# ZeldaM1/PnP-VCVE

Measured on NVIDIA B200. Metric: enhanced_frames_per_sec_720p, higher is better.
Workload: dtype bf16

## Files before the change

### pnpvcve_b200/csrc/pnp_api.cu

```cuda
#include <cmath>
#include <cstddef>
#include <cuda.h>
#include <cuda_runtime.h>
#include <mutex>
#include <stdio.h>
#include <stdlib.h>
#include <string.h>

#include "../../include/pnp_vcve.h"
#include "pnp_conv.cuh"
#include "pnp_ops.cuh"

namespace {

thread_local char g_err[512] = "";
int g_pair_override = -1;

static_assert(sizeof(pnp_dyn_entry) == sizeof(pnp::DynEntry), "launch-table entry layout");

int fail(int code, const char* fmt, const char* detail = "") {
  snprintf(g_err, sizeof(g_err), fmt, detail);
  return code;
}

int cuda_fail(cudaError_t e, const char* where) {
  snprintf(g_err, sizeof(g_err), "%s: %s", where, cudaGetErrorString(e));
  return PNP_ERR_CUDA;
}

struct DeviceInfo {
  bool ok = false;
  int sms = 0;
  int max_pairs = 0;
  cudaError_t err = cudaSuccess;
};

DeviceInfo g_dev[64];
std::once_flag g_dev_once[64];

int device_info(DeviceInfo** out) {
  int dev = 0;
  cudaError_t e = cudaGetDevice(&dev);
  if (e != cudaSuccess) return cuda_fail(e, "cudaGetDevice");
  if (dev < 0 || dev >= 64) return fail(PNP_ERR_ARG, "device ordinal out of range");
  std::call_once(g_dev_once[dev], [dev]() {
    cudaDeviceProp prop;
    cudaError_t e2 = cudaGetDeviceProperties(&prop, dev);
    if (e2 == cudaSuccess) {
      g_dev[dev].ok = (prop.major == 10);
      g_dev[dev].sms = prop.multiProcessorCount;
      if (g_dev[dev].ok) e2 = pnp::conv_rows_prepare(&g_dev[dev].max_pairs);
      if (g_dev[dev].ok && e2 == cudaSuccess) e2 = pnp::warp_prepare();
    }
    g_dev[dev].err = e2;
  });
  *out = &g_dev[dev];
  if (g_dev[dev].err != cudaSuccess) return cuda_fail(g_dev[dev].err, "device initialisation");
  if (!g_dev[dev].ok) return fail(PNP_ERR_ARCH, "libpnpvcve needs an sm_100 device (B200)");
  return PNP_OK;
}

struct Knobs {
  int l2_hints = 0;
  int par_split = 1;
  int warp_tma = 1;
  int pair = 0;
  int rings_nio = 0, rings_sa = 0;
  int debug_skip = 0;
  long long* trace = nullptr;
};

const Knobs& knobs() {
  static const Knobs k = []() {
    Knobs v;
    if (const char* e = getenv("PNP_L2_HINTS")) v.l2_hints = atoi(e);
    if (const char* e = getenv("PNP_PAR_SPLIT")) v.par_split = atoi(e) != 0;
    if (const char* e = getenv("PNP_PAIR")) v.pair = atoi(e);
    if (const char* e = getenv("PNP_WARP_TMA")) v.warp_tma = atoi(e) != 0;
    if (const char* e = getenv("PNP_RINGS")) {
      if (sscanf(e, "%d,%d", &v.rings_nio, &v.rings_sa) != 2) v.rings_nio = v.rings_sa = 0;
    }
#ifdef PNP_DIAG
    if (const char* e = getenv("PNP_DEBUG_SKIP")) v.debug_skip = atoi(e);
    if (const char* e = getenv("PNP_TRACE_PTR")) v.trace = reinterpret_cast<long long*>(strtoull(e, nullptr, 10));
#endif
    return v;
  }();
  return k;
}

pnp::DynRef dyn_ref(const pnp_dyn_ref* d) {
  pnp::DynRef r;
  r.table = d ? reinterpret_cast<const pnp::DynEntry*>(d->table) : nullptr;
  r.step = d ? d->step : nullptr;
  r.node = d ? d->node : 0;
  r.stride = d ? d->stride : 0;
  return r;
}

typedef CUresult (*MemsetD32AsyncFn)(CUdeviceptr, unsigned int, size_t, CUstream);

MemsetD32AsyncFn memset32_fn() {
  static MemsetD32AsyncFn fn = []() -> MemsetD32AsyncFn {
    void* p = nullptr;
    cudaDriverEntryPointQueryResult q;
    if (cudaGetDriverEntryPoint("cuMemsetD32Async", &p, cudaEnableDefault, &q) == cudaSuccess &&
        q == cudaDriverEntryPointSuccess)
      return reinterpret_cast<MemsetD32AsyncFn>(p);
    return nullptr;
  }();
  return fn;
}

int store_step(int32_t* word, int32_t value, cudaStream_t stream) {
  MemsetD32AsyncFn fn = memset32_fn();
  if (fn == nullptr) return fail(PNP_ERR_CUDA, "cuMemsetD32Async entry point not available");
  CUresult r = fn(reinterpret_cast<CUdeviceptr>(word), static_cast<unsigned int>(value), 1, stream);
  if (r != CUDA_SUCCESS) {
    snprintf(g_err, sizeof(g_err), "cuMemsetD32Async failed with CUresult %d", (int)r);
    return PNP_ERR_CUDA;
  }
  return PNP_OK;
}

typedef CUresult (*EncodeTiledFn)(CUtensorMap*, CUtensorMapDataType, cuuint32_t, void*, const cuuint64_t*,
                                  const cuuint64_t*, const cuuint32_t*, const cuuint32_t*,
                                  CUtensorMapInterleave, CUtensorMapSwizzle, CUtensorMapL2promotion,
                                  CUtensorMapFloatOOBfill);

EncodeTiledFn encode_fn() {
  static EncodeTiledFn fn = []() -> EncodeTiledFn {
    void* p = nullptr;
    cudaDriverEntryPointQueryResult q;
    if (cudaGetDriverEntryPoint("cuTensorMapEncodeTiled", &p, cudaEnableDefault, &q) == cudaSuccess &&
        q == cudaDriverEntryPointSuccess)
      return reinterpret_cast<EncodeTiledFn>(p);
    return nullptr;
  }();
  return fn;
}

int make_map(CUtensorMap* m, const void* base, int N, int H, int W, int box_w, long long spx = 0, long long sy = 0,
             long long sn = 0, int box_h = 1, int ch = 64) {
  EncodeTiledFn fn = encode_fn();
  if (fn == nullptr) return fail(PNP_ERR_CUDA, "cuTensorMapEncodeTiled entry point not available");
  const cuuint64_t px = (cuuint64_t)ch * 2;
  cuuint64_t dims[4] = {(cuuint64_t)ch, (cuuint64_t)W, (cuuint64_t)H, (cuuint64_t)N};
  cuuint64_t strides[3] = {px, (cuuint64_t)W * px, (cuuint64_t)H * W * px};
  if (spx != 0) {
    strides[0] = (cuuint64_t)spx * 2;
    strides[1] = (cuuint64_t)sy * 2;
    strides[2] = (cuuint64_t)sn * 2;
  }
  cuuint32_t box[4] = {(cuuint32_t)ch, (cuuint32_t)box_w, (cuuint32_t)box_h, 1};
  cuuint32_t estr[4] = {1, 1, 1, 1};
  CUresult r = fn(m, CU_TENSOR_MAP_DATA_TYPE_BFLOAT16, 4, const_cast<void*>(base), dims, strides, box, estr,
                  CU_TENSOR_MAP_INTERLEAVE_NONE, ch == 32 ? CU_TENSOR_MAP_SWIZZLE_64B : CU_TENSOR_MAP_SWIZZLE_128B,
                  CU_TENSOR_MAP_L2_PROMOTION_L2_256B,
                  CU_TENSOR_MAP_FLOAT_OOB_FILL_NONE);
  if (r != CUDA_SUCCESS) {
    snprintf(g_err, sizeof(g_err), "cuTensorMapEncodeTiled failed with CUresult %d", (int)r);
    return PNP_ERR_CUDA;
  }
  return PNP_OK;
}

bool aligned16(const void* p) { return (reinterpret_cast<uintptr_t>(p) & 15u) == 0; }

int frame_quality(const char* name, const void* a, bool a_u8, int64_t a_sf, int64_t a_sc, int64_t a_sy, const void* b,
                  bool b_u8, int64_t b_sf, int64_t b_sc, int64_t b_sy, int F, int H, int W, int crop_border,
                  unsigned long long* sse, double* ssim_sum, void* stream) {
  if (!a || !b || !sse || !ssim_sum) return fail(PNP_ERR_ARG, "%s: null pointer", name);
  if (F < 1 || crop_border < 0 || H - 2 * crop_border < 11 || W - 2 * crop_border < 11)
    return fail(PNP_ERR_ARG, "%s: the cropped frame must be at least 11 x 11", name);
  if ((long long)F * 3 > 65535) return fail(PNP_ERR_ARG, "%s: at most 21845 frames per call", name);
  DeviceInfo* d;
  int rc = device_info(&d);
  if (rc) return rc;
  double g[11], s = 0.0;
  for (int i = 0; i < 11; ++i) {
    g[i] = exp(-((double)(i - 5) * (i - 5)) / (2.0 * 1.5 * 1.5));
    s += g[i];
  }
  for (int i = 0; i < 11; ++i) g[i] /= s;
  const int ch_first = crop_border != 0 ? 2 : 0, n_ch = crop_border != 0 ? 1 : 3;
  cudaError_t e = pnp::launch_frame_quality(a, a_u8, a_sf, a_sc, a_sy, b, b_u8, b_sf, b_sc, b_sy, F, H, W, crop_border,
                                            ch_first, n_ch, g, sse, ssim_sum, d->sms, static_cast<cudaStream_t>(stream));
  return e == cudaSuccess ? PNP_OK : cuda_fail(e, name);
}

}

extern "C" {

static_assert(sizeof(pnp_conv_desc) == 280 && offsetof(pnp_conv_desc, out_spx) == 184 &&
                  offsetof(pnp_conv_desc, img_off) == 224 && offsetof(pnp_conv_desc, dyn) == 232 &&
                  offsetof(pnp_conv_desc, src_images) == 256 && offsetof(pnp_conv_desc, aux_channels) == 272 &&
                  offsetof(pnp_conv_desc, out_u8) == 276,
              "pnp_conv_desc layout is part of the ABI (mirrored by pnpvcve_b200/_lib.py: ConvDesc)");
int pnp_abi_version(void) { return 10; }

const char* pnp_last_error(void) { return g_err; }

int pnp_device_check(void) {
  DeviceInfo* d;
  return device_info(&d);
}

int pnp_device_pairs(void) {
  DeviceInfo* d;
  int rc = device_info(&d);
  return rc ? rc : d->max_pairs;
}

int pnp_set_pair_mode(int mode) {
  const int prev = g_pair_override;
  g_pair_override = mode < 0 ? -1 : (mode > 2 ? 2 : mode);
  return prev;
}

int pnp_graph_begin(void* stream) {
  DeviceInfo* d;
  int rc = device_info(&d);
  if (rc) return rc;
  cudaError_t e = cudaStreamBeginCapture(static_cast<cudaStream_t>(stream), cudaStreamCaptureModeRelaxed);
  return e == cudaSuccess ? PNP_OK : cuda_fail(e, "pnp_graph_begin");
}

int pnp_graph_end(void* stream, void** graph_exec) {
  if (!graph_exec) return fail(PNP_ERR_ARG, "pnp_graph_end: null output");
  *graph_exec = nullptr;
  cudaGraph_t g = nullptr;
  cudaError_t e = cudaStreamEndCapture(static_cast<cudaStream_t>(stream), &g);
  if (e != cudaSuccess || g == nullptr) {
    if (g) cudaGraphDestroy(g);
    return cuda_fail(e != cudaSuccess ? e : cudaErrorUnknown, "pnp_graph_end: capture");
  }
  cudaGraphExec_t x = nullptr;
  e = cudaGraphInstantiate(&x, g, 0);
  cudaGraphDestroy(g);
  if (e != cudaSuccess) return cuda_fail(e, "pnp_graph_end: instantiate");
  *graph_exec = x;
  return PNP_OK;
}

int pnp_graph_launch(void* graph_exec, int32_t* step_word, int32_t step_value, void* stream) {
  if (!graph_exec) return fail(PNP_ERR_ARG, "pnp_graph_launch: null graph");
  if (step_word) {
    int rc = store_step(step_word, step_value, static_cast<cudaStream_t>(stream));
    if (rc) return rc;
  }
  cudaError_t e = cudaGraphLaunch(static_cast<cudaGraphExec_t>(graph_exec), static_cast<cudaStream_t>(stream));
  return e == cudaSuccess ? PNP_OK : cuda_fail(e, "pnp_graph_launch");
}

int pnp_graph_destroy(void* graph_exec) {
  if (!graph_exec) return PNP_OK;
  cudaError_t e = cudaGraphExecDestroy(static_cast<cudaGraphExec_t>(graph_exec));
  return e == cudaSuccess ? PNP_OK : cuda_fail(e, "pnp_graph_destroy");
}

int pnp_set_step(int32_t* step_word, int32_t step_value, void* stream) {
  if (!step_word) return fail(PNP_ERR_ARG, "pnp_set_step: null step word");
  return store_step(step_word, step_value, static_cast<cudaStream_t>(stream));
}

int pnp_fetch_pinned(void* dst, const void* src_pinned, int64_t bytes, void* stream) {
  if (!dst || !src_pinned) return fail(PNP_ERR_ARG, "pnp_fetch_pinned: null pointer");
  if (bytes < 0 || (bytes & 15) || !aligned16(dst) || !aligned16(src_pinned))
    return fail(PNP_ERR_ARG, "pnp_fetch_pinned: size and pointers must be multiples of 16 bytes");
  DeviceInfo* d;
  int rc = device_info(&d);
  if (rc) return rc;
  cudaPointerAttributes at;
  cudaError_t e = cudaPointerGetAttributes(&at, src_pinned);
  if (e != cudaSuccess) return cuda_fail(e, "pnp_fetch_pinned");
  if (at.type != cudaMemoryTypeHost || at.devicePointer == nullptr)
    return fail(PNP_ERR_ARG, "pnp_fetch_pinned: src must be page-locked host memory the device can address");
  e = pnp::launch_fetch_pinned(at.devicePointer, dst, bytes, static_cast<cudaStream_t>(stream));
  return e == cudaSuccess ? PNP_OK : cuda_fail(e, "pnp_fetch_pinned");
}

int pnp_mv_warp(const void* src, const float* flow_x, const float* flow_y, int64_t flow_row_stride,
                int64_t flow_image_stride, void* dst, int N, int H, int W, int32_t* dbg_x0, int32_t* dbg_y0,
                void* stream) {
  if (!src || !flow_x || !flow_y || !dst) return fail(PNP_ERR_ARG, "pnp_mv_warp: null pointer");
  if (N <= 0 || H < 10 || W < 10) return fail(PNP_ERR_ARG, "pnp_mv_warp: bad shape (images of at least 10 x 10 pixels)");
  if (!aligned16(src) || !aligned16(dst) || src == dst)
    return fail(PNP_ERR_ARG, "pnp_mv_warp: src/dst must be distinct 16-byte aligned buffers");
  if ((dbg_x0 == nullptr) != (dbg_y0 == nullptr) || (dbg_x0 && N != 1))
    return fail(PNP_ERR_ARG, "pnp_mv_warp: dbg outputs come in pairs and need N == 1");
  DeviceInfo* d;
  int rc = device_info(&d);
  if (rc) return rc;
  CUtensorMap tm, tmd;
  if ((rc = make_map(&tm, src, N, H, W, 10, 0, 0, 0, 10))) return rc;
  if ((rc = make_map(&tmd, dst, N, H, W, 8, 0, 0, 0, 8))) return rc;
  cudaError_t e = pnp::launch_mv_warp(tm, tmd, src, flow_x, flow_y, flow_row_stride, flow_image_stride, dst, N, H, W, dbg_x0,
                                      dbg_y0, dyn_ref(nullptr), nullptr, knobs().warp_tma, static_cast<cudaStream_t>(stream));
  return e == cudaSuccess ? PNP_OK : cuda_fail(e, "pnp_mv_warp");
}

int pnp_mv_warp_dyn(const pnp_dyn_ref* dyn, const void* src_pool, int src_pool_images, int64_t flow_row_stride,
                    int64_t flow_image_stride, int N, int H, int W, void* stream) {
  if (!dyn || !dyn->table || !dyn->step) return fail(PNP_ERR_ARG, "pnp_mv_warp_dyn: null launch table");
  if (N <= 0 || H < 10 || W < 10) return fail(PNP_ERR_ARG, "pnp_mv_warp_dyn: bad shape (images of at least 10 x 10 pixels)");
  if (!src_pool || src_pool_images < N || !aligned16(src_pool))
    return fail(PNP_ERR_ARG, "pnp_mv_warp_dyn: src_pool must be the 16-byte aligned buffer every table entry's src lies in");
  DeviceInfo* d;
  int rc = device_info(&d);
  if (rc) return rc;
  CUtensorMap tm, tmd;
  if ((rc = make_map(&tm, src_pool, src_pool_images, H, W, 10, 0, 0, 0, 10))) return rc;
  if ((rc = make_map(&tmd, src_pool, src_pool_images, H, W, 8, 0, 0, 0, 8))) return rc;
  cudaError_t e = pnp::launch_mv_warp(tm, tmd, nullptr, nullptr, nullptr, flow_row_stride, flow_image_stride, nullptr, N, H, W,
                                      nullptr, nullptr, dyn_ref(dyn), src_pool, knobs().warp_tma,
                                      static_cast<cudaStream_t>(stream));
  return e == cudaSuccess ? PNP_OK : cuda_fail(e, "pnp_mv_warp_dyn");
}

int pnp_lr_im2col(const float* lr, int64_t sn, int64_t sc, int64_t sy, void* dst, int N, int H, int W,
                  int dst_channels, void* stream) {
  if (!lr || !dst) return fail(PNP_ERR_ARG, "pnp_lr_im2col: null pointer");
  if (N <= 0 || H <= 0 || W <= 0 || !aligned16(dst) || (dst_channels != 64 && dst_channels != 32))
    return fail(PNP_ERR_ARG, "pnp_lr_im2col: bad argument (dst_channels is 64 or 32)");
  DeviceInfo* d;
  int rc = device_info(&d);
  if (rc) return rc;
  cudaError_t e = pnp::launch_lr_im2col(lr, sn, sc, sy, dst, N, H, W, dst_channels, dyn_ref(nullptr),
                                        static_cast<cudaStream_t>(stream));
  return e == cudaSuccess ? PNP_OK : cuda_fail(e, "pnp_lr_im2col");
}

int pnp_lr_im2col_dyn(const pnp_dyn_ref* dyn, int64_t sn, int64_t sc, int64_t sy, int N, int H, int W, int dst_channels,
                      void* stream) {
  if (!dyn || !dyn->table || !dyn->step) return fail(PNP_ERR_ARG, "pnp_lr_im2col_dyn: null launch table");
  if (N <= 0 || H <= 0 || W <= 0 || (dst_channels != 64 && dst_channels != 32))
    return fail(PNP_ERR_ARG, "pnp_lr_im2col_dyn: bad shape (dst_channels is 64 or 32)");
  DeviceInfo* d;
  int rc = device_info(&d);
  if (rc) return rc;
  cudaError_t e = pnp::launch_lr_im2col(nullptr, sn, sc, sy, nullptr, N, H, W, dst_channels, dyn_ref(dyn),
                                        static_cast<cudaStream_t>(stream));
  return e == cudaSuccess ? PNP_OK : cuda_fail(e, "pnp_lr_im2col_dyn");
}

int pnp_pack_conv3x3_rowstack(const float* w, int n_experts, const float* coef, const float* row_scale,
                              int out_ch, int in_total, int in_begin, int in_begin2, int in_count, void* dst,
                              int tap_n, int flip_ky, void* stream) {
  if (!w || !dst) return fail(PNP_ERR_ARG, "pnp_pack_conv3x3_rowstack: null pointer");
  if (n_experts < 1 || (coef == nullptr && n_experts != 1) || out_ch < 1 || (tap_n != 64 && tap_n != 16) ||
      out_ch > tap_n || in_count < 1 || in_count > 64 || in_begin < 0 || in_begin + in_count > in_total ||
      (in_begin2 >= 0 && in_begin2 + in_count > in_total) || !aligned16(dst))
    return fail(PNP_ERR_ARG, "pnp_pack_conv3x3_rowstack: bad argument");
  DeviceInfo* d;
  int rc = device_info(&d);
  if (rc) return rc;
  cudaError_t e = pnp::launch_pack_conv3x3_rowstack(w, n_experts, coef, row_scale, out_ch, in_total, in_begin, in_begin2,
                                                    in_count, dst, tap_n, flip_ky != 0, static_cast<cudaStream_t>(stream));
  return e == cudaSuccess ? PNP_OK : cuda_fail(e, "pnp_pack_conv3x3_rowstack");
}

int pnp_pack_rows(const float* w, int rows, int cols, int64_t row_stride, int64_t col_stride, void* dst,
                  int row_offset, void* stream) {
  if (!w || !dst) return fail(PNP_ERR_ARG, "pnp_pack_rows: null pointer");
  if (rows < 1 || rows > 64 || cols < 1 || cols > 64 || row_offset < 0 || !aligned16(dst))
    return fail(PNP_ERR_ARG, "pnp_pack_rows: bad argument");
  DeviceInfo* d;
  int rc = device_info(&d);
  if (rc) return rc;
  cudaError_t e = pnp::launch_pack_rows(w, rows, cols, row_stride, col_stride, dst, row_offset,
                                        static_cast<cudaStream_t>(stream));
  return e == cudaSuccess ? PNP_OK : cuda_fail(e, "pnp_pack_rows");
}

int pnp_pack_aux(const float* w, int out_ch, int in_total, void* dst, void* stream) {
  if (!w || !dst) return fail(PNP_ERR_ARG, "pnp_pack_aux: null pointer");
  if (out_ch < 1 || out_ch > 64 || in_total < 3 || !aligned16(dst))
    return fail(PNP_ERR_ARG, "pnp_pack_aux: bad argument");
  DeviceInfo* d;
  int rc = device_info(&d);
  if (rc) return rc;
  cudaError_t e = pnp::launch_pack_aux(w, out_ch, in_total, dst, static_cast<cudaStream_t>(stream));
  return e == cudaSuccess ? PNP_OK : cuda_fail(e, "pnp_pack_aux");
}

int pnp_pack_mix_blocks(const float* w2, const float* w1x1, int n_blocks, int n_experts, const float* coef,
                        const float* row_scale, void* dst, int64_t dst_block_stride, void* stream) {
  if (!w2 || !w1x1 || !coef || !row_scale || !dst) return fail(PNP_ERR_ARG, "pnp_pack_mix_blocks: null pointer");
  if (n_blocks < 1 || n_blocks > 65535 || n_experts < 1 || dst_block_stride < 12 * 8192 || (dst_block_stride & 15) ||
      !aligned16(dst))
    return fail(PNP_ERR_ARG, "pnp_pack_mix_blocks: bad argument");
  DeviceInfo* d;
  int rc = device_info(&d);
  if (rc) return rc;
  cudaError_t e = pnp::launch_pack_mix_blocks(w2, w1x1, n_blocks, n_experts, coef, row_scale, dst, dst_block_stride,
                                              static_cast<cudaStream_t>(stream));
  return e == cudaSuccess ? PNP_OK : cuda_fail(e, "pnp_pack_mix_blocks");
}

int pnp_caa_heads(const float* base_qp, const float* qp, int frames, const float* base0_w,
                  const float* base0_b, const float* base2_w, const float* base2_b, const float* se0_w,
                  const float* se2_w, int n_experts, int se_hidden, float* experts, float* gamma,
                  void* stream) {
  if (!base_qp || !qp || !base0_w || !base0_b || !base2_w || !base2_b || !se0_w || !se2_w || !experts || !gamma)
    return fail(PNP_ERR_ARG, "pnp_caa_heads: null pointer");
  if (frames < 1 || n_experts < 1 || n_experts > 16 || se_hidden < 1 || se_hidden > 64)
    return fail(PNP_ERR_ARG, "pnp_caa_heads: bad argument");
  DeviceInfo* d;
  int rc = device_info(&d);
  if (rc) return rc;
  cudaError_t e = pnp::launch_caa_heads(base_qp, qp, frames, base0_w, base0_b, base2_w, base2_b, se0_w, se2_w,
                                        n_experts, se_hidden, experts, gamma, static_cast<cudaStream_t>(stream));
  return e == cudaSuccess ? PNP_OK : cuda_fail(e, "pnp_caa_heads");
}

int pnp_mix_bias(const float* conv2_bias, int n_blocks, int n_experts, const float* experts,
                 const float* gamma, int frames, float* out, void* stream) {
  if (!conv2_bias || !experts || !gamma || !out) return fail(PNP_ERR_ARG, "pnp_mix_bias: null pointer");
  if (n_blocks < 1 || n_blocks > 65535 || n_experts < 1 || frames < 1)
    return fail(PNP_ERR_ARG, "pnp_mix_bias: bad argument");
  DeviceInfo* d;
  int rc = device_info(&d);
  if (rc) return rc;
  cudaError_t e = pnp::launch_mix_bias(conv2_bias, (long long)n_experts * 64, n_blocks, n_experts, experts, gamma,
                                       frames, out, static_cast<cudaStream_t>(stream));
  return e == cudaSuccess ? PNP_OK : cuda_fail(e, "pnp_mix_bias");
}

int pnp_mv_rasterize(const float* records, const int32_t* frame_offsets, const int32_t* is_b,
                     const int32_t* p_target, int T, int R, int H, int W, uint32_t* owner_fwd,
                     uint32_t* owner_bwd, uint32_t* part_mask, float* mvs, float* partitions,
                     int32_t* status, void* stream) {
  if (!frame_offsets || !is_b || !p_target || !owner_fwd || !owner_bwd || !part_mask || !mvs || !partitions ||
      !status || (R > 0 && !records))
    return fail(PNP_ERR_ARG, "pnp_mv_rasterize: null pointer");
  if (T < 1 || T > 65535 || R < 0 || H < 1 || H > 65535 || W < 1 || (long long)T * H * W >= (1LL << 31))
    return fail(PNP_ERR_ARG, "pnp_mv_rasterize: bad shape");
  DeviceInfo* d;
  int rc = device_info(&d);
  if (rc) return rc;
  cudaError_t e = pnp::launch_mv_rasterize(records, frame_offsets, is_b, p_target, T, R, H, W, owner_fwd, owner_bwd,
                                           part_mask, mvs, partitions, status, static_cast<cudaStream_t>(stream));
  return e == cudaSuccess ? PNP_OK : cuda_fail(e, "pnp_mv_rasterize");
}

int pnp_frame_quality(const float* a, int64_t a_sf, int64_t a_sc, int64_t a_sy, const float* b, int64_t b_sf,
                      int64_t b_sc, int64_t b_sy, int F, int H, int W, int crop_border, unsigned long long* sse,
                      double* ssim_sum, void* stream) {
  return frame_quality("pnp_frame_quality", a, false, a_sf, a_sc, a_sy, b, false, b_sf, b_sc, b_sy, F, H, W, crop_border,
                       sse, ssim_sum, stream);
}

int pnp_frame_quality_u8(const void* a, int a_is_u8, int64_t a_sf, int64_t a_sc, int64_t a_sy, const void* b,
                         int b_is_u8, int64_t b_sf, int64_t b_sc, int64_t b_sy, int F, int H, int W, int crop_border,
                         unsigned long long* sse, double* ssim_sum, void* stream) {
  return frame_quality("pnp_frame_quality_u8", a, a_is_u8 != 0, a_sf, a_sc, a_sy, b, b_is_u8 != 0, b_sf, b_sc, b_sy, F,
                       H, W, crop_border, sse, ssim_sum, stream);
}

int pnp_unit_from_u8(const uint8_t* src, int64_t s_sf, int64_t s_sc, int64_t s_sy, float* dst, int64_t d_sf,
                     int64_t d_sc, int64_t d_sy, int F, int H, int W, void* stream) {
  if (!src || !dst) return fail(PNP_ERR_ARG, "pnp_unit_from_u8: null pointer");
  if (F < 1 || F > 65535 || H < 1 || H > 21845 || W < 1)
    return fail(PNP_ERR_ARG, "pnp_unit_from_u8: bad shape (1 <= F <= 65535, 1 <= H <= 21845)");
  DeviceInfo* d;
  int rc = device_info(&d);
  if (rc) return rc;
  cudaError_t e = pnp::launch_unit_from_u8(src, s_sf, s_sc, s_sy, dst, d_sf, d_sc, d_sy, F, H, W,
                                           static_cast<cudaStream_t>(stream));
  return e == cudaSuccess ? PNP_OK : cuda_fail(e, "pnp_unit_from_u8");
}

int pnp_conv3x3(const pnp_conv_desc* c, void* stream) {
  if (!c) return fail(PNP_ERR_ARG, "pnp_conv3x3: null descriptor");
  const bool table = c->dyn.table != nullptr;
  if (!c->src || (!table && !c->wpack)) return fail(PNP_ERR_ARG, "pnp_conv3x3: null src/wpack");
  if (table && (!c->dyn.step || c->dyn.node < 0 || c->dyn.stride <= c->dyn.node))
    return fail(PNP_ERR_ARG, "pnp_conv3x3: bad launch-table reference");
  if (c->N < 1 || c->H < 8 || c->W < 1) return fail(PNP_ERR_ARG, "pnp_conv3x3: bad shape (at least 8 rows)");
  const bool last = (c->mode == PNP_CONV_LAST);
  if (c->mode != PNP_CONV_BF16 && !last) return fail(PNP_ERR_ARG, "pnp_conv3x3: bad mode");
  const bool par = c->par != nullptr;
  if (last) {
    if (!c->lq || !c->outf || c->tap_n != 16 || c->aux || c->idt || par)
      return fail(PNP_ERR_ARG, "pnp_conv3x3: PNP_CONV_LAST needs lq/outf, tap_n=16, no aux/idt/par");
  } else {
    if (!c->out || c->tap_n != 64) return fail(PNP_ERR_ARG, "pnp_conv3x3: PNP_CONV_BF16 needs out and tap_n=64");
    if (c->out == c->src && !table) return fail(PNP_ERR_ARG, "pnp_conv3x3: out must not alias src (halo rows)");
  }
  if ((c->aux != nullptr) != (c->aux_k16 > 0) || c->aux_k16 < 0 || c->aux_k16 > 4)
    return fail(PNP_ERR_ARG, "pnp_conv3x3: aux / aux_k16 mismatch");
  const bool aux32 = c->aux && c->aux_channels == 32;
  if (c->aux && c->aux_channels != 0 && c->aux_channels != 64 && !aux32)
    return fail(PNP_ERR_ARG, "pnp_conv3x3: aux_channels is 64 (or 0) or 32");
  if (aux32 && c->aux_k16 > 2) return fail(PNP_ERR_ARG, "pnp_conv3x3: a 32-channel aux source carries K <= 32");
  if (par && (c->aux || c->idt)) return fail(PNP_ERR_ARG, "pnp_conv3x3: par takes no aux / idt");
  if (c->act < 0 || c->act > 2) return fail(PNP_ERR_ARG, "pnp_conv3x3: bad act");
  const bool strided_out = c->out_spx != 0 || c->out_sy != 0 || c->out_sn != 0;
  if (strided_out && (last || c->out_spx < 64 || c->out_sy < c->out_spx * c->W || (c->N > 1 && c->out_sn < c->out_sy * c->H) ||
                      ((c->out_spx | c->out_sy | c->out_sn) & 7)))
    return fail(PNP_ERR_ARG, "pnp_conv3x3: out strides must be non-overlapping multiples of 8 elements (PNP_CONV_BF16 only)");
  if (c->out_u8 && !last) return fail(PNP_ERR_ARG, "pnp_conv3x3: out_u8 needs PNP_CONV_LAST");
  if (c->lq_up4 && (!last || (c->H & 3) || (c->W & 3)))
    return fail(PNP_ERR_ARG, "pnp_conv3x3: lq_up4 needs PNP_CONV_LAST and H, W multiples of 4");
  if (!aligned16(c->src) || (c->wpack && !aligned16(c->wpack)) || (c->aux && !aligned16(c->aux)) ||
      (c->idt && !aligned16(c->idt)) || (c->out && !aligned16(c->out)))
    return fail(PNP_ERR_ARG, "pnp_conv3x3: pointers must be 16-byte aligned");
  if (c->src_images < 0 || c->aux_images < 0 || c->idt_images < 0 || c->out_images < 0)
    return fail(PNP_ERR_ARG, "pnp_conv3x3: negative image count");
  DeviceInfo* d;
  int rc = device_info(&d);
  if (rc) return rc;
  if (c->per_image && (c->N > d->sms || (!table && !c->img_off)))
    return fail(PNP_ERR_ARG, "pnp_conv3x3: per_image needs img_off and at most one image per SM");

  const Knobs& kn = knobs();
  pnp::ConvParams p;
  memset(&p, 0, sizeof(p));
  auto images = [&](int32_t n) { return n > 0 ? n : c->N; };
  if ((rc = make_map(&p.tm_src, c->src, images(c->src_images), c->H, c->W, pnp::kHaloPx))) return rc;
  if (c->aux && (rc = make_map(&p.tm_aux, c->aux, images(c->aux_images), c->H, c->W, pnp::kTilePx, 0, 0, 0, 1,
                               aux32 ? 32 : 64)))
    return rc;
  if (c->idt && (rc = make_map(&p.tm_id, c->idt, images(c->idt_images), c->H, c->W, pnp::kTilePx))) return rc;
  if (!last && (rc = make_map(&p.tm_out, c->out, images(c->out_images), c->H, c->W, pnp::kTilePx, c->out_spx, c->out_sy,
                              c->out_sn)))
    return rc;
  if (last) p.tm_out = p.tm_src;
  p.dyn = dyn_ref(&c->dyn);
  p.wpack = c->wpack;
  p.scale = c->scale;
  p.bias = c->bias;
  p.has_bias = c->bias != nullptr;
  p.img_off = c->per_image ? reinterpret_cast<const long long*>(c->img_off) : nullptr;
  p.par = c->par;
  p.has_par = par ? 1 : 0;
  p.par_sn = c->par_sn; p.par_sc = c->par_sc; p.par_sy = c->par_sy;
  p.lq = c->lq;
  p.lq_sn = c->lq_sn; p.lq_sc = c->lq_sc; p.lq_sy = c->lq_sy;
  p.outf = c->outf;
  p.of_sn = c->of_sn; p.of_sc = c->of_sc; p.of_sy = c->of_sy;
  p.out_u8 = c->out_u8 ? 1 : 0;
  p.H = c->H; p.W = c->W; p.N = c->N;
  p.strips = (c->W + pnp::kTilePx - 1) / pnp::kTilePx;
  const long long tiles = (long long)c->N * p.strips * c->H;
  if (tiles > 0x7fffffffLL) return fail(PNP_ERR_ARG, "pnp_conv3x3: too many tiles");
  p.tiles_total = (int)tiles;
  const long long cols = (long long)c->N * p.strips;
  const int pair_mode = g_pair_override >= 0 ? g_pair_override : kn.pair;
  const bool pair_ok = pair_mode != 0 && !last && !aux32 && c->tap_n == 64 && d->max_pairs >= 8 && (!par || kn.par_split) &&
                       (c->per_image ? (p.strips % 2 == 0 && c->N <= d->max_pairs)
                                     : (cols % 2 == 0 || cols >= 15 || pair_mode == 2));
  int grid;
  if (pair_ok) {
    p.pair = 1;
    const int max_pairs = d->max_pairs < d->sms / 2 ? d->max_pairs : d->sms / 2;
    if (c->per_image) {
      const int tiles_img = (p.strips / 2) * c->H;
      int cpi = max_pairs / c->N;
      if (cpi > tiles_img) cpi = tiles_img;
      p.tiles_per_cta = (tiles_img + cpi - 1) / cpi;
      cpi = (tiles_img + p.tiles_per_cta - 1) / p.tiles_per_cta;
      p.cpi = cpi;
      p.tiles_total = tiles_img * c->N;
      grid = 2 * cpi * c->N;
    } else {
      const long long pair_tiles = ((cols + 1) / 2) * c->H;
      p.tiles_total = (int)pair_tiles;
      int clusters = max_pairs < pair_tiles ? max_pairs : (int)pair_tiles;
      p.tiles_per_cta = (p.tiles_total + clusters - 1) / clusters;
      clusters = (p.tiles_total + p.tiles_per_cta - 1) / p.tiles_per_cta;
      grid = 2 * clusters;
    }
  } else if (c->per_image) {
    const int tiles_img = p.strips * c->H;
    int cpi = d->sms / c->N;
    if (cpi > tiles_img) cpi = tiles_img;
    p.tiles_per_cta = (tiles_img + cpi - 1) / cpi;
    cpi = (tiles_img + p.tiles_per_cta - 1) / p.tiles_per_cta;
    p.cpi = cpi;
    grid = cpi * c->N;
  } else {
    grid = d->sms < p.tiles_total ? d->sms : p.tiles_total;
    p.tiles_per_cta = (p.tiles_total + grid - 1) / grid;
    grid = (p.tiles_total + p.tiles_per_cta - 1) / p.tiles_per_cta;
  }
  p.tap_n = c->tap_n;
  p.aux_k16 = c->aux_k16;
  p.aux_pitch64 = aux32 ? 1 : 0;
  p.has_id = c->idt != nullptr;
  p.act = c->act;
  p.mode = last ? pnp::kModeLast : pnp::kModeBf16;
  p.flip_y = c->flip_y ? 1 : 0;
  p.w_stable = c->wpack_stable ? 1 : 0;
  p.lq_up4 = c->lq_up4 ? 1 : 0;
  p.par_sparse = (par && c->par_sparse) ? 1 : 0;
  if (kn.l2_hints && c->idt && c->flip_y) {
    p.l2_src = p.l2_idt = 1;
    if (kn.l2_hints >= 2) p.l2_out = 2;
  } else if (kn.l2_hints >= 2 && par) {
    p.l2_src = kn.l2_hints == 2 ? 2 : 1;
    p.l2_out = kn.l2_hints == 2 ? 1 : 2;
  }
  p.par_split = (par && kn.par_split) ? 1 : 0;
  p.debug_skip = kn.debug_skip;
  p.trace = kn.trace;
  const long long budget = 232448 - 2048;
  const long long w_bytes = ((long long)9 * c->tap_n * 128 + (c->aux ? pnp::kWChunkBytes : 0) / (p.pair ? 2 : 1) +
                             (par ? 3 * 64 * 128 : 0) / (p.pair ? 2 : 1) + 1023) & ~1023LL;
  auto fixed_bytes = [&](int n_io) {
    return w_bytes + (c->aux ? 2 * pnp::kTileBytes : 0) + (long long)n_io * pnp::kTileBytes;
  };
  p.n_io = 2;
  if (par) p.n_io = 3;
  if (c->idt) {
    p.n_io = 4;
    while (p.n_io > 2 && (budget - fixed_bytes(p.n_io)) / pnp::kASlotBytes < 5) --p.n_io;
  }
  long long slots = (budget - fixed_bytes(p.n_io)) / pnp::kASlotBytes;
  const long long max_slots = 6;
  if (slots > max_slots) slots = max_slots;
  if (slots < 4) return fail(PNP_ERR_RESOURCE, "pnp_conv3x3: shared-memory budget cannot hold 4 source rows");
  if (c->idt && p.n_io < 3)
    return fail(PNP_ERR_RESOURCE, "pnp_conv3x3: idt needs 3 staging slots (drop aux)");
  p.s_a = (int)slots;
  if (kn.rings_nio >= 2 && kn.rings_nio <= pnp::kMaxIoSlots && kn.rings_sa >= 3 && kn.rings_sa <= pnp::kMaxASlots &&
      fixed_bytes(kn.rings_nio) + (long long)kn.rings_sa * pnp::kASlotBytes <= budget && !(c->idt && kn.rings_nio < 3) &&
      !(par && kn.rings_nio < 3)) {
    p.n_io = kn.rings_nio;
    p.s_a = kn.rings_sa;
  }
  cudaError_t e = pnp::launch_conv_rows(p, grid, static_cast<cudaStream_t>(stream));
  return e == cudaSuccess ? PNP_OK : cuda_fail(e, "pnp_conv3x3");
}

}
```

### pnpvcve_b200/csrc/pnp_conv.cuh

```cuda
#pragma once
#include <cuda.h>
#include <stdint.h>

namespace pnp {

constexpr int kTilePx = 128;
constexpr int kHaloPx = kTilePx + 2;
constexpr int kRowBytes = kHaloPx * 128;
constexpr int kASlotBytes = 17 * 1024;
constexpr int kTileBytes = kTilePx * 128;
constexpr int kWChunkBytes = 8192;
constexpr int kRowsThreads = 352;
constexpr int kRowsThreadsPar = 480;
constexpr int kEpilogueWarps = 8;
constexpr int kMaxASlots = 8;
constexpr int kMaxIoSlots = 6;
constexpr int kTmemCols = 512;

enum ConvMode { kModeBf16 = 0, kModeLast = 1 };
enum ConvAct { kActNone = 0, kActLrelu = 1, kActRelu = 2 };

struct DynEntry {
  unsigned long long p[6];
  int i[4];
};
static_assert(sizeof(DynEntry) == 64, "launch-table entry is 64 bytes (ABI)");

struct DynRef {
  const DynEntry* table;
  const int* step;
  int node, stride;
  __device__ __forceinline__ const DynEntry* entry() const {
    return table ? table + ((long long)(*step) * stride + node) : nullptr;
  }
};

struct ConvParams {
  CUtensorMap tm_src;
  CUtensorMap tm_aux;
  CUtensorMap tm_id;
  CUtensorMap tm_out;
  DynRef dyn;
  const void* wpack;
  const float* scale;
  const float* bias;
  const long long* img_off;
  const float* par;
  long long par_sn, par_sc, par_sy;
  const float* lq;
  long long lq_sn, lq_sc, lq_sy;
  float* outf;
  long long of_sn, of_sc, of_sy;
  int H, W, N, strips;
  int tiles_total, tiles_per_cta;
  int cpi;
  int has_par;
  int has_bias;
  int tap_n;
  int aux_k16;
  int aux_pitch64;
  int has_id;
  int act;
  int mode;
  int flip_y;
  int l2_src, l2_idt, l2_out;
  int par_split;
  int par_sparse;
  int lq_up4;
  int w_stable;
  int pair;
  int s_a;
  int n_io;
  long long* trace;
  int debug_skip;
  int out_u8;
};

__device__ __forceinline__ void par_sparse_select(float& p0, float& p1, float& p2) {
  const bool n2 = p2 != 0.f, n1 = p1 != 0.f, n0 = p0 != 0.f;
  const float c = 1.0f / 255.0f;
  p2 = n2 ? c : 0.f;
  p1 = (!n2 && n1) ? c : 0.f;
  p0 = (!n2 && !n1 && n0) ? c : 0.f;
}

size_t conv_rows_smem_bytes(const ConvParams& p);
cudaError_t conv_rows_prepare(int* max_pairs);
cudaError_t launch_conv_rows(const ConvParams& p, int grid, cudaStream_t stream);

}
```

### pnpvcve_b200/csrc/pnp_conv_rows.cu

```cuda
#include <type_traits>

#include "pnp_conv.cuh"
#include "pnp_ops.cuh"
#include "pnp_ptx.cuh"

#ifdef PNP_DIAG
#define PNP_DBG(bit) ((p.debug_skip & (bit)) != 0)
#define PNP_TRACING (p.trace != nullptr)
#else
#define PNP_DBG(bit) false
#define PNP_TRACING false
#endif

namespace pnp {

namespace {

constexpr int kAccRingMax = 8;
#ifndef PNP_STEP_RING_LOG2
#define PNP_STEP_RING_LOG2 4
#endif
constexpr int kStepShift = PNP_STEP_RING_LOG2;
constexpr int kStepRing = 1 << kStepShift;
constexpr int kParCol = 320;

struct RowsLayout {
  uint32_t w, a, aux, io, misc, total;
};

__host__ __device__ inline RowsLayout rows_layout(int w_bytes, int s_a, int has_aux, int n_io) {
  RowsLayout l;
  l.w = 0;
  l.a = l.w + ((w_bytes + 1023) & ~1023);
  l.aux = l.a + s_a * kASlotBytes;
  l.io = l.aux + (has_aux ? 2 * kTileBytes : 0);
  l.misc = l.io + n_io * kTileBytes;
  l.total = l.misc + 1024;
  return l;
}

struct RowsMisc {
  float scale[64];
  float bias[64];
  uint64_t w_full;
  uint64_t a_full[kMaxASlots];
  uint64_t step_done[kStepRing];
  uint64_t acc_free[kAccRingMax];
  uint64_t par_done;
  uint64_t aux_full[2];
  uint64_t id_full[kMaxIoSlots];
  uint64_t io_empty[kMaxIoSlots];
  uint32_t tmem_base;
  uint32_t go_step;
  uint32_t go_par;
  uint32_t slot_free;
  uint64_t dy_full[kMaxIoSlots];
  uint64_t peer_w;
};
static_assert(sizeof(RowsMisc) <= 1024, "misc region overflow");

struct Segment {
  int n, strip, y_b, len, j_first, j_last;
};

struct SegIter {
  int t, t_end, H, strips, n, strip, y_b, dcol;
  __device__ SegIter(const ConvParams& p, int b, int e, int rank = 0) : t(b), t_end(e), H(p.H), strips(p.strips) {
    int col = b / p.H;
    y_b = b - col * p.H;
    dcol = p.pair ? 2 : 1;
    if (p.pair) col = 2 * col + rank;
    n = col / p.strips;
    strip = col - n * p.strips;
  }
  __device__ __forceinline__ bool valid() const { return t < t_end; }
  __device__ __forceinline__ Segment get() const {
    Segment s;
    s.n = n;
    s.strip = strip;
    s.y_b = y_b;
    s.len = min(H - y_b, t_end - t);
    s.j_first = (y_b > 0) ? -1 : 0;
    s.j_last = (y_b + s.len < H) ? s.len : s.len - 1;
    return s;
  }
  __device__ __forceinline__ void next(const Segment& s) {
    t += s.len;
    y_b = 0;
    strip += dcol;
    while (strip >= strips) {
      strip -= strips;
      ++n;
    }
  }
};

struct Ring {
  uint32_t slot, phase, size;
  __device__ explicit Ring(uint32_t n) : slot(0), phase(0), size(n) {}
  __device__ __forceinline__ void advance() {
    if (++slot == size) {
      slot = 0;
      phase ^= 1;
    }
  }
};

__device__ __forceinline__ float act_fn(float v, int act) {
  if (act == kActLrelu) return v > 0.f ? v : 0.1f * v;
  if (act == kActRelu) return fmaxf(v, 0.f);
  return v;
}

}

template <bool kPar, bool kScale, bool kPair>
__global__ void __launch_bounds__(kPar ? kRowsThreadsPar : kRowsThreads, 1)
conv3x3_rows_kernel(const __grid_constant__ ConvParams p) {
  constexpr int kAccRing = kPar ? 5 : 8;
  const int rank = kPair ? (int)cluster_ctarank() : 0;
  const int unit = kPair ? (int)(blockIdx.x >> 1) : (int)blockIdx.x;
  extern __shared__ uint8_t smem_raw[];
  const uint32_t raw = smem_u32(smem_raw);
  const uint32_t sbase = (raw + 1023u) & ~1023u;
  uint8_t* sgen = smem_raw + (sbase - raw);
  const int tap_n = p.tap_n;
  const int dx_block_bytes = 3 * tap_n * 128;
  const int w_bytes = kPair ? 3 * dx_block_bytes + (p.aux_k16 > 0 ? kWChunkBytes / 2 : 0) + (kPar ? 3 * 64 * 128 / 2 : 0)
                            : 3 * dx_block_bytes + (p.aux_k16 > 0 ? kWChunkBytes : 0) + (kPar ? 3 * 64 * 128 : 0);
  const RowsLayout L = rows_layout(w_bytes, p.s_a, p.aux_k16 > 0, p.n_io);
  RowsMisc* misc = reinterpret_cast<RowsMisc*>(sgen + L.misc);

  const int warp = threadIdx.x >> 5;
  const int lane = threadIdx.x & 31;
  int t_begin, t_end, img = 0;
  if (p.cpi > 0) {
    img = unit / p.cpi;
    const int tiles_img = (kPair ? p.strips >> 1 : p.strips) * p.H;
    t_begin = img * tiles_img + (unit - img * p.cpi) * p.tiles_per_cta;
    t_end = min((img + 1) * tiles_img, t_begin + p.tiles_per_cta);
  } else {
    t_begin = unit * p.tiles_per_cta;
    t_end = min(p.tiles_total, t_begin + p.tiles_per_cta);
  }
  const DynEntry* dyn = p.dyn.entry();
  const long long* img_off = dyn ? reinterpret_cast<const long long*>(dyn->p[5]) : p.img_off;
  const long long w_off = img_off ? img_off[2 * img] : 0, b_off = img_off ? img_off[2 * img + 1] : 0;
  const uint8_t* const wpack = (dyn ? reinterpret_cast<const uint8_t*>(dyn->p[0]) : static_cast<const uint8_t*>(p.wpack)) + w_off;
  const float* const bias_g = p.has_bias ? (dyn ? reinterpret_cast<const float*>(dyn->p[1]) : p.bias) + b_off : nullptr;
  const float* const par_g = dyn ? reinterpret_cast<const float*>(dyn->p[2]) : p.par;
  const float* const lq_g = dyn ? reinterpret_cast<const float*>(dyn->p[3]) : p.lq;
  float* const outf_g = dyn ? reinterpret_cast<float*>(dyn->p[4]) : p.outf;
  const int src_f = dyn ? dyn->i[0] : 0, aux_f = dyn ? dyn->i[1] : 0, idt_f = dyn ? dyn->i[2] : 0,
            out_f = dyn ? dyn->i[3] : 0;
  const int s_a = p.s_a;
  const int n_io = p.n_io;
  const bool last_mode = (p.mode == kModeLast);
  const int y_flip_base = p.flip_y ? p.H - 1 : 0;
  const int y_sign = p.flip_y ? -1 : 1;
#define PNP_Y(yy) (y_flip_base + y_sign * (yy))

  if (threadIdx.x < 64) {
    misc->scale[threadIdx.x] = p.scale ? p.scale[threadIdx.x] : 1.0f;
    const int nb = last_mode ? 3 : 64;
    misc->bias[threadIdx.x] = (bias_g && threadIdx.x < nb) ? bias_g[threadIdx.x] : 0.0f;
  }
  if (warp == 0) {
    if (lane == 0) {
      mbar_init(smem_u32(&misc->w_full), 1);
      for (int i = 0; i < kMaxASlots; ++i) mbar_init(smem_u32(&misc->a_full[i]), 1);
      for (int i = 0; i < kStepRing; ++i) mbar_init(smem_u32(&misc->step_done[i]), 1);
      const int acc_readers = kEpilogueWarps * (kPair ? 2 : 1);
      for (int i = 0; i < kAccRingMax; ++i) mbar_init(smem_u32(&misc->acc_free[i]), acc_readers);
      mbar_init(smem_u32(&misc->peer_w), 1);
      for (int i = 0; i < kMaxIoSlots; ++i) mbar_init(smem_u32(&misc->dy_full[i]), 4);
      misc->slot_free = 0;
      mbar_init(smem_u32(&misc->par_done), 1);
      for (int i = 0; i < 2; ++i) mbar_init(smem_u32(&misc->aux_full[i]), 1);
      for (int i = 0; i < kMaxIoSlots; ++i) {
        mbar_init(smem_u32(&misc->id_full[i]), 1);
        mbar_init(smem_u32(&misc->io_empty[i]), 1);
      }
      misc->go_step = 0;
      misc->go_par = 0;
      mbar_fence_init();
      tma_prefetch_desc(&p.tm_src);
      if (!last_mode) tma_prefetch_desc(&p.tm_out);
    }
    __syncwarp();
    if (kPair) tmem_alloc2(smem_u32(&misc->tmem_base), kTmemCols);
    else tmem_alloc(smem_u32(&misc->tmem_base), kTmemCols);
  }
  tc_fence_before();
  if (kPair) cluster_sync_all(); else __syncthreads();
  tc_fence_after();
  const uint32_t tmem_base = misc->tmem_base;
  griddep_launch_dependents();
  const uint32_t w_smem_early = sbase + L.w;
  auto load_weights = [&]() {
    const uint32_t wbar = smem_u32(&misc->w_full);
    mbar_arrive_expect_tx(wbar, w_bytes);
    if (kPair) {
      const int h192 = dx_block_bytes >> 1, h64 = (tap_n * 128) >> 1;
      for (int dx = 0; dx < 3; ++dx)
        bulk_load_1d(w_smem_early + dx * h192, wpack + dx * dx_block_bytes + rank * h192, h192, wbar);
      for (int b = 0; b < 9; ++b)
        bulk_load_1d(w_smem_early + 3 * h192 + b * h64, wpack + b * (tap_n * 128) + rank * h64, h64, wbar);
      const int extra = w_bytes - 3 * dx_block_bytes;
      if (extra > 0)
        bulk_load_1d(w_smem_early + 3 * dx_block_bytes, wpack + 3 * dx_block_bytes + rank * extra, extra, wbar);
    } else {
      for (int off = 0; off < w_bytes; off += kWChunkBytes) {
        const int n = min(kWChunkBytes, w_bytes - off);
        bulk_load_1d(w_smem_early + off, wpack + off, n, wbar);
      }
    }
  };
  if (p.w_stable && warp == 0) {
    if (elect_one()) load_weights();
    __syncwarp();
  }
  griddep_wait();
  if (PNP_TRACING && threadIdx.x == 0) {
    p.trace[2048 + blockIdx.x] = -clock64();
    p.trace[2208 + blockIdx.x] = (long long)globaltimer_ns();
  }
  const bool par_defer = kPar && p.par_split && PNP_DBG(1024);
  const bool hot_waits = !PNP_DBG(32);
  const uint32_t hint_ns = PNP_DBG(64) ? 40u : 200u;
  auto pwait = [&](uint32_t bar, uint32_t parity, int tag) {
    if (hot_waits) mbar_wait(bar, parity, tag); else mbar_wait_patient(bar, parity, tag, hint_ns);
  };
  auto ewait = [&](uint32_t bar, uint32_t parity, int tag) {
    if (hot_waits) mbar_wait(bar, parity, tag); else mbar_wait_warp(bar, parity, tag, hint_ns);
  };
  auto slow_epilogue = [&]() {
    if (PNP_DBG(2048)) __nanosleep(2000);
  };
  const uint32_t w_smem = sbase + L.w;
  const uint32_t a_smem = sbase + L.a;
  const uint32_t aux_smem = sbase + L.aux;
  const uint32_t io_smem = sbase + L.io;

  if (warp == 0) {
    if (elect_one()) {
      if (!p.w_stable) load_weights();
      const uint64_t pol_src = p.l2_src == 2 ? l2_policy_evict_last() : l2_policy_evict_first();
      Ring ar(s_a);
      uint32_t sc = 0, ord = 0;
      uint32_t aux_step[2] = {0, 0};
      for (SegIter it(p, t_begin, t_end, rank); it.valid();) {
        const Segment s = it.get();
        const int x0 = s.strip * kTilePx;
        for (int j = s.j_first; j <= s.j_last; ++j, ++sc, ar.advance()) {
          if (sc >= (uint32_t)s_a) {
            const uint32_t ps = sc - s_a + (par_defer ? 1u : 0u);
            pwait(smem_u32(&misc->step_done[ps & (kStepRing - 1)]), (ps >> kStepShift) & 1, 1);
          }
          const uint32_t fb = smem_u32(&misc->a_full[ar.slot]);
          if (kPair) {
            if (rank == 0) mbar_arrive_expect_tx(fb, 2 * kRowBytes);
            tma_load_4d_pair(a_smem + ar.slot * kASlotBytes, &p.tm_src, mapa_shared(fb, 0), 0, x0 - 1, PNP_Y(s.y_b + j),
                             s.n + src_f);
          } else if (PNP_DBG(1) && sc >= (uint32_t)s_a) {
            mbar_arrive(fb);
          } else {
            mbar_arrive_expect_tx(fb, kRowBytes);
            if (p.l2_src)
              tma_load_4d_hint(a_smem + ar.slot * kASlotBytes, &p.tm_src, fb, 0, x0 - 1, PNP_Y(s.y_b + j), s.n + src_f, pol_src);
            else
              tma_load_4d(a_smem + ar.slot * kASlotBytes, &p.tm_src, fb, 0, x0 - 1, PNP_Y(s.y_b + j), s.n + src_f);
          }
          if (j >= 0 && j < s.len) {
            if (p.aux_k16 > 0) {
              const uint32_t as = ord & 1;
              if (ord >= 2) {
                const uint32_t ps = aux_step[as];
                pwait(smem_u32(&misc->step_done[ps & (kStepRing - 1)]), (ps >> kStepShift) & 1, 2);
              }
              aux_step[as] = sc;
              const uint32_t ab = smem_u32(&misc->aux_full[as]);
              if (kPair) {
                if (rank == 0) mbar_arrive_expect_tx(ab, 2 * kTileBytes);
                tma_load_4d_pair(aux_smem + as * kTileBytes, &p.tm_aux, mapa_shared(ab, 0), 0, x0, PNP_Y(s.y_b + j),
                                 s.n + aux_f);
              } else {
                mbar_arrive_expect_tx(ab, p.aux_pitch64 ? kTileBytes / 2 : kTileBytes);
                tma_load_4d(aux_smem + as * kTileBytes, &p.tm_aux, ab, 0, x0, PNP_Y(s.y_b + j), s.n + aux_f);
              }
            }
            ++ord;
          }
        }
        it.next(s);
      }
    }
  } else if (warp == 1) {
    if (kPair && rank != 0) {
      if (elect_one()) {
        mbar_wait(smem_u32(&misc->w_full), 0, 4);
        mbar_arrive_cluster(mapa_shared(smem_u32(&misc->peer_w), 0));
      }
    } else if (elect_one()) {
      const uint32_t idesc0 = umma_idesc_bf16(kPair ? 256 : 128, 0);
      const uint32_t idesc_step = ((uint32_t)tap_n >> 3) << 17;
      const uint32_t w_lo = umma_desc_lo(w_smem);
      const uint32_t dxb = (uint32_t)dx_block_bytes >> 4;
      const uint32_t sbb = (uint32_t)(tap_n * 128) >> 4;
      const uint32_t aux_w_lo = w_lo + 3 * dxb;
      const uint32_t aux_a_hi = p.aux_pitch64 ? kDescHiSw64 : kDescHiSw128;
      const uint32_t par_w_lo = w_lo + 3 * dxb;
      const uint32_t u192 = dxb >> 1, u64 = sbb >> 1, w64_lo = w_lo + 3 * (dxb >> 1);
      mbar_wait(smem_u32(&misc->w_full), 0, 4);
      if (kPair) mbar_wait(smem_u32(&misc->peer_w), 0, 14);
      struct StepCtx {
        bool valid;
        int j, len, j_first;
        uint32_t ord0, sc, a_slot, a_phase;
      };
      SegIter seg_it(p, t_begin, t_end, rank);
      Segment seg = seg_it.valid() ? seg_it.get() : Segment{0, 0, 0, 0, 0, -1};
      Ring ar(s_a);
      StepCtx cur{seg_it.valid(), seg.j_first, seg.len, seg.j_first, 0u, 0u, ar.slot, ar.phase};
      auto advance = [&](StepCtx& c) {
        ar.advance();
        c.sc += 1;
        c.a_slot = ar.slot;
        c.a_phase = ar.phase;
        if (c.j < seg.j_last) {
          c.j += 1;
          return;
        }
        const uint32_t next_ord0 = c.ord0 + (uint32_t)seg.len;
        seg_it.next(seg);
        c.valid = seg_it.valid();
        if (c.valid) {
          seg = seg_it.get();
          c.j = seg.j_first;
          c.len = seg.len;
          c.j_first = seg.j_first;
          c.ord0 = next_ord0;
        }
      };
      auto ranges = [](const StepCtx& c, int& lo, int& cnt, int& old_cnt) {
        lo = max(c.j - 1, 0);
        const int hi = min(c.j + 1, c.len - 1);
        cnt = hi - lo + 1;
        const int new_from = (c.j == c.j_first) ? lo : c.j + 1;
        old_cnt = min(max(new_from - lo, 0), cnt);
      };
      const uint32_t go_step = smem_u32(&misc->go_step), go_par = smem_u32(&misc->go_par);
      bool pend = false;
      uint32_t pend_bar = 0;
      auto commit = [&](uint32_t bar) {
        if (kPair) umma2_commit(bar); else umma_commit(bar);
      };

      auto mma_range = [&](auto wrap_tag, uint32_t slot_lo, int cnt, uint32_t a_lo, uint32_t b_lo, uint32_t acc) {
        constexpr bool kWrap = decltype(wrap_tag)::value;
        if constexpr (!kWrap) {
          umma_bf16_lo(tmem_base + slot_lo * tap_n, a_lo, kDescHiSw128, b_lo, kDescHiSw128, idesc0 + cnt * idesc_step, acc);
        } else {
          const int n1 = min(cnt, kAccRing - (int)slot_lo);
          if (cnt > n1) {
            umma1_bf16_lo<1>(tmem_base + slot_lo * tap_n, a_lo, b_lo, idesc0 + n1 * idesc_step, acc);
            umma1_bf16_lo<3>(tmem_base, a_lo, b_lo + n1 * sbb, idesc0 + (cnt - n1) * idesc_step, acc);
          } else {
            umma_bf16_lo(tmem_base + slot_lo * tap_n, a_lo, kDescHiSw128, b_lo, kDescHiSw128, idesc0 + n1 * idesc_step, acc);
          }
        }
      };

      bool ppend = false;
      uint32_t pp_arow = 0, pp_od = 0;
      auto issue_par = [&](uint32_t a_row_, uint32_t od) {
        const uint32_t readers = (p.par_split ? 4u : (uint32_t)kEpilogueWarps) * (kPair ? 2u : 1u);
        if (kPair) {
          uint32_t spins = 0;
          while (ld_volatile_shared(go_par) < readers * od) {
            if (++spins > PNP_SPIN_LIMIT) {
              printf("pnp: flag wait timed out (tag 10, block %d, target %u)\n", (int)blockIdx.x, readers * od);
              __trap();
            }
          }
        } else {
          spin_until_ge(go_par, readers * od, 10);
        }
        tc_fence_after();
#pragma unroll
        for (int k = 0; k < 4; ++k) {
          if (kPair)
            umma2_bf16_lo<0>(tmem_base + kParCol, a_row_ + 8 + 2 * k, par_w_lo + 2 * k, idesc0 + 3 * idesc_step, k > 0);
          else
            umma_bf16_lo(tmem_base + kParCol, a_row_ + 8 + 2 * k, kDescHiSw128, par_w_lo + 2 * k, kDescHiSw128,
                         idesc0 + 3 * idesc_step, k > 0);
        }
        commit(smem_u32(&misc->par_done));
      };

      uint32_t go_seen = 0;
      const bool dbg_nopoll = PNP_DBG(8), dbg_nofence = PNP_DBG(16);
      if (cur.valid) go_seen = spin_until_ge_v(go_step, 1, 5);
      tc_fence_after();
      while (cur.valid) {
        const bool tr = PNP_TRACING && blockIdx.x == 0 && cur.sc < 64 && !PNP_DBG(128);
        if (tr) p.trace[cur.sc * 8 + 0] = clock64();
        int lo, cnt, old_cnt;
        ranges(cur, lo, cnt, old_cnt);
        const int new_cnt = cnt - old_cnt;
        const bool centre = (cur.j >= 0 && cur.j < cur.len);
        const uint32_t slot_lo = (cur.ord0 + lo) % kAccRing;
        const uint32_t a_row = umma_desc_lo(a_smem + cur.a_slot * kASlotBytes);
        const uint32_t sb_lo = (uint32_t)(lo - (cur.j - 1));
        const uint32_t b_row = w_lo + sb_lo * sbb;
        const uint32_t cur_sc = cur.sc;
        const uint32_t cur_od = cur.ord0 + (uint32_t)max(cur.j, 0);
        StepCtx nxt = cur;
        advance(nxt);
        auto step_body = [&](auto emit) {
#pragma unroll
          for (int dx = 0; dx < 3; ++dx) {
            if (kPar && dx == 1 && ppend) {
              issue_par(pp_arow, pp_od);
              ppend = false;
            }
            if (tr && dx == 1) p.trace[cur_sc * 8 + 6] = clock64();
            if (dx == 2) {
              if (tr) p.trace[cur_sc * 8 + 7] = clock64();
              if (nxt.valid && go_seen < nxt.sc + 1 && !dbg_nopoll) {
                go_seen = spin_until_ge_v(go_step, nxt.sc + 1, 5);
                if (!dbg_nofence) tc_fence_after();
              }
              if (tr) p.trace[cur_sc * 8 + 2] = clock64();
            }
#pragma unroll
            for (int k = 0; k < 4; ++k) {
              emit(dx, k);
              if (dx == 0 && k == 0 && pend) {
                commit(pend_bar);
                pend = false;
              }
              if (tr) p.trace[1024 + cur_sc * 16 + dx * 4 + k] = clock64();
            }
          }
        };
        if constexpr (kPair) {
          uint32_t dcol[3];
#pragma unroll
          for (int i = 0; i < 3; ++i) {
            uint32_t sl = slot_lo + (uint32_t)i;
            if (sl >= (uint32_t)kAccRing) sl -= (uint32_t)kAccRing;
            dcol[i] = tmem_base + sl * tap_n;
          }
          const uint32_t idesc_sb = idesc0 + idesc_step, idesc_win = idesc0 + 3 * idesc_step;
          auto rows = [&](auto cnt_tag, int dx, int k, uint32_t a_lo, bool first) {
            constexpr int kCnt = decltype(cnt_tag)::value;
            const uint32_t b0 = w64_lo + ((uint32_t)dx * 3 + sb_lo) * u64 + 2 * k;
            const uint32_t acc0 = first ? (old_cnt > 0) : 1u, acc1 = first ? (old_cnt > 1) : 1u,
                           acc2 = first ? (old_cnt > 2) : 1u;
            if constexpr (kCnt == 1) {
              umma2_bf16_lo<0>(dcol[0], a_lo, b0, idesc_sb, acc0);
            } else if constexpr (kCnt == 2) {
              umma2_bf16_lo<1>(dcol[0], a_lo, b0, idesc_sb, acc0);
              umma2_bf16_lo<3>(dcol[1], a_lo, b0 + u64, idesc_sb, acc1);
            } else {
              umma2_bf16_lo<1>(dcol[0], a_lo, b0, idesc_sb, acc0);
              umma2_bf16_lo<2>(dcol[1], a_lo, b0 + u64, idesc_sb, acc1);
              umma2_bf16_lo<3>(dcol[2], a_lo, b0 + 2 * u64, idesc_sb, acc2);
            }
          };
          if (cnt == 3 && slot_lo + 3u <= (uint32_t)kAccRing) {
            step_body([&](int dx, int k) {
              const uint32_t a_lo = a_row + dx * 8 + 2 * k;
              if (dx == 0 && k == 0) rows(std::integral_constant<int, 3>{}, dx, k, a_lo, true);
              else umma2_bf16_lo<0>(dcol[0], a_lo, w_lo + (uint32_t)dx * u192 + 2 * k, idesc_win, 1);
            });
          } else if (cnt == 3) {
            step_body([&](int dx, int k) {
              rows(std::integral_constant<int, 3>{}, dx, k, a_row + dx * 8 + 2 * k, dx == 0 && k == 0);
            });
          } else if (cnt == 2) {
            step_body([&](int dx, int k) {
              rows(std::integral_constant<int, 2>{}, dx, k, a_row + dx * 8 + 2 * k, dx == 0 && k == 0);
            });
          } else {
            step_body([&](int dx, int k) {
              rows(std::integral_constant<int, 1>{}, dx, k, a_row + dx * 8 + 2 * k, dx == 0 && k == 0);
            });
          }
        } else {
          auto emit1 = [&](auto wrap_tag, int dx, int k) {
            const uint32_t a_lo = a_row + dx * 8 + 2 * k;
            const uint32_t b_lo = b_row + dx * dxb + 2 * k;
            if (dx == 0 && k == 0) {
              if (old_cnt > 0) mma_range(wrap_tag, slot_lo, old_cnt, a_lo, b_lo, 1);
              if (new_cnt > 0)
                mma_range(wrap_tag, (slot_lo + old_cnt) % kAccRing, new_cnt, a_lo, b_lo + old_cnt * sbb, 0);
            } else {
              mma_range(wrap_tag, slot_lo, cnt, a_lo, b_lo, 1);
            }
          };
          if (slot_lo + (uint32_t)cnt > (uint32_t)kAccRing)
            step_body([&](int dx, int k) { emit1(std::true_type{}, dx, k); });
          else
            step_body([&](int dx, int k) { emit1(std::false_type{}, dx, k); });
        }
        if (p.aux_k16 > 0 && centre) {
          const uint32_t a_lo = umma_desc_lo(aux_smem + (cur_od & 1) * kTileBytes);
          for (int k = 0; k < p.aux_k16; ++k) {
            if (kPair)
              umma2_bf16_lo<0>(tmem_base + (cur_od % kAccRing) * tap_n, a_lo + 2 * k, aux_w_lo + 2 * k,
                               idesc0 + idesc_step, 1);
            else
              umma_bf16_lo(tmem_base + (cur_od % kAccRing) * tap_n, a_lo + 2 * k, aux_a_hi,
                           aux_w_lo + 2 * k, kDescHiSw128, idesc0 + idesc_step, 1);
          }
        }
        if (kPar && centre) {
          if (par_defer) {
            ppend = true;
            pp_arow = a_row;
            pp_od = cur_od;
          } else {
            issue_par(a_row, cur_od);
          }
        }
        pend = true;
        pend_bar = smem_u32(&misc->step_done[cur_sc & (kStepRing - 1)]);
        if (tr) p.trace[cur_sc * 8 + 1] = clock64();
        cur = nxt;
      }
      if (kPar && ppend) issue_par(pp_arow, pp_od);
      if (pend) commit(pend_bar);
    }
  } else if (warp == 10) {
    if ((!kPair || rank == 0) && elect_one()) {
      const uint32_t go_step = smem_u32(&misc->go_step);
      Ring ar(s_a);
      uint32_t sc = 0, ord0 = 0;
      for (SegIter it(p, t_begin, t_end, rank); it.valid();) {
        const Segment s = it.get();
        for (int j = s.j_first; j <= s.j_last; ++j, ++sc, ar.advance()) {
          const bool trs = PNP_TRACING && blockIdx.x == 0 && sc < 64;
          if (trs) p.trace[2560 + sc * 4 + 0] = clock64();
          mbar_wait(smem_u32(&misc->a_full[ar.slot]), ar.phase, 5);
          if (trs) p.trace[2560 + sc * 4 + 1] = clock64();
          const int lo = max(j - 1, 0), hi = min(j + 1, s.len - 1);
          const int new_from = (j == s.j_first) ? lo : j + 1;
          for (int o = max(new_from, lo); o <= hi; ++o) {
            const uint32_t od = ord0 + o;
            mbar_wait(smem_u32(&misc->acc_free[od % kAccRing]), ((od / kAccRing) & 1) ^ 1, 6);
          }
          const bool centre = (j >= 0 && j < s.len);
          if (p.aux_k16 > 0 && centre) {
            const uint32_t od = ord0 + j;
            mbar_wait(smem_u32(&misc->aux_full[od & 1]), (od >> 1) & 1, 7);
          }
          st_release_shared(go_step, sc + 1);
          if (trs) p.trace[2560 + sc * 4 + 2] = clock64();
        }
        ord0 += s.len;
        it.next(s);
      }
    }
  } else if (warp >= 11 && !(kPar && p.par_split)) {
  } else {
    const int q = warp & 3;
    const int half = (warp - 2) >> 2;
    const int row = q * 32 + lane;
    const bool store_warp = (warp == 2);
    const uint32_t sw = (uint32_t)(row & 7);
    const uint32_t lane_base = tmem_base + ((uint32_t)(q * 32) << 16);
    float bias_r[kPar ? 1 : 32], scale_r[(kScale && !kPar) ? 32 : 1];
    if (!kPar) {
#pragma unroll
      for (int j = 0; j < 32; ++j) {
        bias_r[j] = misc->bias[half * 32 + j];
        if (kScale) scale_r[j] = misc->scale[half * 32 + j];
      }
    }

    struct TileCur {
      SegIter it;
      Segment s;
      int o;
      uint32_t ord, sc0;
      bool valid;
    };
    TileCur cur{SegIter(p, t_begin, t_end, rank), Segment{0, 0, 0, 0, 0, -1}, 0, 0u, 0u, false};
    cur.valid = cur.it.valid();
    if (cur.valid) cur.s = cur.it.get();
    const uint32_t acc_free0 = kPair ? mapa_shared(smem_u32(&misc->acc_free[0]), 0) : smem_u32(&misc->acc_free[0]);
    const uint32_t go_par_a = kPair ? mapa_shared(smem_u32(&misc->go_par), 0) : smem_u32(&misc->go_par);
    auto acc_release = [&](uint32_t slot) {
      __syncwarp();
      if (lane == 0) {
        if (kPair) mbar_arrive_cluster(acc_free0 + slot * 8);
        else mbar_arrive(acc_free0 + slot * 8);
      }
    };
    auto par_release = [&]() {
      __syncwarp();
      if (lane == 0) {
        if (kPair) red_add_cluster(go_par_a);
        else asm volatile("red.relaxed.cta.shared::cta.add.u32 [%0], 1;" ::"r"(go_par_a) : "memory");
      }
    };
    auto phantom = [&](const Segment& sg) { return kPair && sg.n >= p.N; };
    auto tile_next = [](TileCur& c) {
      ++c.ord;
      if (++c.o < c.s.len) return;
      c.sc0 += (uint32_t)(c.s.j_last - c.s.j_first + 1);
      c.it.next(c.s);
      c.valid = c.it.valid();
      c.o = 0;
      if (c.valid) c.s = c.it.get();
    };

    auto blend_store = [&](uint8_t* slot_row, float q0, float q1, float q2) {
      if (p.par_sparse) par_sparse_select(q0, q1, q2);
#pragma unroll
      for (int gg = 0; gg < 2; ++gg) {
        float a1[16], a2[16], a3[16];
        const uint32_t col = kParCol + half * 32 + gg * 16;
        tmem_ld16(lane_base + col, a1);
        tmem_ld16(lane_base + col + 64, a2);
        tmem_ld16(lane_base + col + 128, a3);
        tmem_ld_wait();
        uint32_t w[8];
#pragma unroll
        for (int j = 0; j < 8; ++j)
          w[j] = pack_bf16x2(fmaf(q2, a3[2 * j], fmaf(q1, a2[2 * j], q0 * a1[2 * j])),
                             fmaf(q2, a3[2 * j + 1], fmaf(q1, a2[2 * j + 1], q0 * a1[2 * j + 1])));
        const int g = half * 2 + gg;
        *reinterpret_cast<uint4*>(slot_row + (((2 * g) ^ sw) << 4)) = make_uint4(w[0], w[1], w[2], w[3]);
        *reinterpret_cast<uint4*>(slot_row + (((2 * g + 1) ^ sw) << 4)) = make_uint4(w[4], w[5], w[6], w[7]);
      }
    };
    auto par_load = [&](const TileCur& c, float& q0, float& q1, float& q2) {
      const int x = c.s.strip * kTilePx + row;
      q0 = q1 = q2 = 0.f;
      if (x < p.W && !phantom(c.s)) {
        const float* pp = par_g + (long long)c.s.n * p.par_sn + (long long)PNP_Y(c.s.y_b + c.o) * p.par_sy + x;
        q0 = __ldg(pp);
        q1 = __ldg(pp + p.par_sc);
        q2 = __ldg(pp + 2 * p.par_sc);
      }
    };
    if (kPar && p.par_split) {
      const uint32_t slot_free = smem_u32(&misc->slot_free);
      if (warp >= 11) {
        float pn0 = 0.f, pn1 = 0.f, pn2 = 0.f;
        if (cur.valid) par_load(cur, pn0, pn1, pn2);
        Ring sl(n_io);
        while (cur.valid) {
          TileCur nxt = cur;
          tile_next(nxt);
          float pf0 = 0.f, pf1 = 0.f, pf2 = 0.f;
          if (nxt.valid) par_load(nxt, pf0, pf1, pf2);
          const bool trr = PNP_TRACING && blockIdx.x == 0 && cur.ord < 64 && warp == 11 && lane == 0;
          if (trr) p.trace[3072 + cur.ord * 4 + 0] = clock64();
          mbar_wait(smem_u32(&misc->par_done), cur.ord & 1, 11);
          if (trr) p.trace[3072 + cur.ord * 4 + 1] = clock64();
          tc_fence_after();
          if (p.par_sparse) par_sparse_select(pn0, pn1, pn2);
          uint32_t wv[32];
#pragma unroll
          for (int b4 = 0; b4 < 4; ++b4) {
            float a1[16], a2[16], a3[16];
            const uint32_t col = kParCol + b4 * 16;
            tmem_ld16(lane_base + col, a1);
            tmem_ld16(lane_base + col + 64, a2);
            tmem_ld16(lane_base + col + 128, a3);
            tmem_ld_wait();
            if (b4 == 3) {
              tc_fence_before();
              par_release();
              if (trr) p.trace[3072 + cur.ord * 4 + 2] = clock64();
            }
#pragma unroll
            for (int j = 0; j < 8; ++j)
              wv[b4 * 8 + j] = pack_bf16x2(fmaf(pn2, a3[2 * j], fmaf(pn1, a2[2 * j], pn0 * a1[2 * j])),
                                           fmaf(pn2, a3[2 * j + 1], fmaf(pn1, a2[2 * j + 1], pn0 * a1[2 * j + 1])));
          }
          if (cur.ord >= (uint32_t)n_io) spin_until_ge(slot_free, cur.ord - (uint32_t)n_io + 1, 12);
          uint8_t* rowp = sgen + L.io + sl.slot * kTileBytes + row * 128;
#pragma unroll
          for (int c8 = 0; c8 < 8; ++c8)
            *reinterpret_cast<uint4*>(rowp + ((c8 ^ sw) << 4)) =
                make_uint4(wv[4 * c8], wv[4 * c8 + 1], wv[4 * c8 + 2], wv[4 * c8 + 3]);
          warp_arrive(smem_u32(&misc->dy_full[sl.slot]));
          if (trr) p.trace[3072 + cur.ord * 4 + 3] = clock64();
          sl.advance();
          pn0 = pf0;
          pn1 = pf1;
          pn2 = pf2;
          cur = nxt;
        }
      } else {
        Ring ior(n_io);
        while (cur.valid) {
          const Segment& s = cur.s;
          const uint32_t ord = cur.ord;
          const int y = PNP_Y(s.y_b + cur.o);
          const uint32_t sc_last = cur.sc0 + (uint32_t)(min(cur.o + 1, s.j_last) - s.j_first);
          const uint32_t slot = ord % kAccRing;
          const uint32_t taddr = lane_base + slot * tap_n;
          if (store_warp) {
            if (elect_one()) {
              tma_store_wait_read<1>();
              if (ord >= 1) st_release_shared(slot_free, ord - 1);
            }
            __syncwarp();
          }
          const bool trm = PNP_TRACING && blockIdx.x == 0 && ord < 64 && warp == 2 && lane == 0;
          if (trm) p.trace[2816 + ord * 4 + 0] = clock64();
          slow_epilogue();
          mbar_wait(smem_u32(&misc->step_done[sc_last & (kStepRing - 1)]), (sc_last >> kStepShift) & 1, 9);
          if (trm) p.trace[2816 + ord * 4 + 1] = clock64();
          tc_fence_after();
          float v[32];
          tmem_ld16(taddr + half * 32, v);
          tmem_ld16(taddr + half * 32 + 16, v + 16);
          tmem_ld_wait();
          tc_fence_before();
          acc_release(slot);
          if (trm) p.trace[2816 + ord * 4 + 2] = clock64();
          mbar_wait(smem_u32(&misc->dy_full[ior.slot]), ior.phase, 13);
          if (trm) p.trace[2816 + ord * 4 + 3] = clock64();
          uint8_t* rowp = sgen + L.io + ior.slot * kTileBytes + row * 128;
#pragma unroll
          for (int gg = 0; gg < 2; ++gg) {
            const int g = half * 2 + gg;
            float* vv = v + gg * 16;
            const float4* sc4 = reinterpret_cast<const float4*>(&misc->scale[g * 16]);
            const float4* bi4 = reinterpret_cast<const float4*>(&misc->bias[g * 16]);
#pragma unroll
            for (int j4 = 0; j4 < 4; ++j4) {
              const float4 sc = kScale ? sc4[j4] : make_float4(1.f, 1.f, 1.f, 1.f);
              const float4 bi = bi4[j4];
              vv[4 * j4 + 0] = fmaf(vv[4 * j4 + 0], sc.x, bi.x);
              vv[4 * j4 + 1] = fmaf(vv[4 * j4 + 1], sc.y, bi.y);
              vv[4 * j4 + 2] = fmaf(vv[4 * j4 + 2], sc.z, bi.z);
              vv[4 * j4 + 3] = fmaf(vv[4 * j4 + 3], sc.w, bi.w);
            }
            uint4* c0 = reinterpret_cast<uint4*>(rowp + (((2 * g) ^ sw) << 4));
            uint4* c1 = reinterpret_cast<uint4*>(rowp + (((2 * g + 1) ^ sw) << 4));
            const uint4 i0 = *c0, i1 = *c1;
            const uint32_t iw[8] = {i0.x, i0.y, i0.z, i0.w, i1.x, i1.y, i1.z, i1.w};
#pragma unroll
            for (int j = 0; j < 8; ++j) {
              vv[2 * j] += bf16_lo(iw[j]);
              vv[2 * j + 1] += bf16_hi(iw[j]);
            }
#pragma unroll
            for (int j = 0; j < 16; ++j) vv[j] = act_fn(vv[j], p.act);
            *c0 = make_uint4(pack_bf16x2(vv[0], vv[1]), pack_bf16x2(vv[2], vv[3]), pack_bf16x2(vv[4], vv[5]),
                             pack_bf16x2(vv[6], vv[7]));
            *c1 = make_uint4(pack_bf16x2(vv[8], vv[9]), pack_bf16x2(vv[10], vv[11]), pack_bf16x2(vv[12], vv[13]),
                             pack_bf16x2(vv[14], vv[15]));
          }
          fence_proxy_async_smem();
          named_bar_sync(2, 256);
          if (store_warp) {
            if (elect_one()) {
              if (!phantom(s)) {
                if (p.l2_out)
                  tma_store_4d_hint(&p.tm_out, io_smem + ior.slot * kTileBytes, 0, s.strip * kTilePx, y, s.n + out_f,
                                    p.l2_out == 2 ? l2_policy_evict_last() : l2_policy_evict_first());
                else
                  tma_store_4d(&p.tm_out, io_smem + ior.slot * kTileBytes, 0, s.strip * kTilePx, y, s.n + out_f);
              }
              tma_store_commit();
            }
            __syncwarp();
          }
          ior.advance();
          tile_next(cur);
        }
        if (store_warp) {
          if (elect_one()) tma_store_wait_all<0>();
          __syncwarp();
        }
      }
    } else {
    float pn0 = 0.f, pn1 = 0.f, pn2 = 0.f;
    if (kPar && cur.valid) {
      float q0, q1, q2;
      par_load(cur, q0, q1, q2);
      {
        TileCur n1 = cur;
        tile_next(n1);
        if (n1.valid) par_load(n1, pn0, pn1, pn2);
      }
      ewait(smem_u32(&misc->par_done), cur.ord & 1, 11);
      tc_fence_after();
      blend_store(sgen + L.io + row * 128, q0, q1, q2);
      tc_fence_before();
      par_release();
    }

    TileCur idc = cur;
    Ring idr(n_io);
    auto load_id = [&](const TileCur& c, uint32_t slot) {
      const uint32_t ib = smem_u32(&misc->id_full[slot]);
      mbar_arrive_expect_tx(ib, kTileBytes);
      if (p.l2_idt)
        tma_load_4d_hint(io_smem + slot * kTileBytes, &p.tm_id, ib, 0, c.s.strip * kTilePx, PNP_Y(c.s.y_b + c.o), c.s.n + idt_f,
                         p.l2_idt == 2 ? l2_policy_evict_last() : l2_policy_evict_first());
      else
        tma_load_4d(io_smem + slot * kTileBytes, &p.tm_id, ib, 0, c.s.strip * kTilePx, PNP_Y(c.s.y_b + c.o), c.s.n + idt_f);
    };
    if (p.has_id && store_warp) {
      if (elect_one()) {
        for (int i = 0; i < n_io && idc.valid; ++i) {
          load_id(idc, idr.slot);
          idr.advance();
          tile_next(idc);
        }
      }
      __syncwarp();
    }

    auto lq_fetch = [&](const TileCur& c, float* r) {
      r[0] = r[1] = r[2] = 0.f;
      if (!c.valid || half != 0) return;
      const int x = c.s.strip * kTilePx + row;
      const int y = PNP_Y(c.s.y_b + c.o);
      if (x >= p.W) return;
      if (p.lq_up4) {
        const int hl = p.H >> 2, wl = p.W >> 2;
        const float sy = fmaxf(0.25f * ((float)y + 0.5f) - 0.5f, 0.f), sx = fmaxf(0.25f * ((float)x + 0.5f) - 0.5f, 0.f);
        const int y0 = (int)sy, x0 = (int)sx;
        const int y1 = y0 + (y0 < hl - 1 ? 1 : 0), x1 = x0 + (x0 < wl - 1 ? 1 : 0);
        const float ly1 = sy - (float)y0, lx1 = sx - (float)x0;
        const float ly0 = 1.f - ly1, lx0 = 1.f - lx1;
        const float* b0 = lq_g + (long long)c.s.n * p.lq_sn + (long long)y0 * p.lq_sy;
        const float* b1 = lq_g + (long long)c.s.n * p.lq_sn + (long long)y1 * p.lq_sy;
#pragma unroll
        for (int ch = 0; ch < 3; ++ch) {
          const float* c0 = b0 + ch * p.lq_sc;
          const float* c1 = b1 + ch * p.lq_sc;
          r[ch] = ly0 * (lx0 * __ldg(c0 + x0) + lx1 * __ldg(c0 + x1)) + ly1 * (lx0 * __ldg(c1 + x0) + lx1 * __ldg(c1 + x1));
        }
      } else {
        const float* lp = lq_g + (long long)c.s.n * p.lq_sn + (long long)y * p.lq_sy + x;
        r[0] = __ldg(lp);
        r[1] = __ldg(lp + p.lq_sc);
        r[2] = __ldg(lp + 2 * p.lq_sc);
      }
    };
    float lq_a[3] = {0.f, 0.f, 0.f}, lq_b[3] = {0.f, 0.f, 0.f};
    if (last_mode) {
      lq_fetch(cur, lq_a);
      TileCur n1 = cur;
      if (n1.valid) tile_next(n1);
      lq_fetch(n1, lq_b);
    }

    Ring ior(n_io);
    while (cur.valid) {
      slow_epilogue();
      const Segment& s = cur.s;
      const int o = cur.o;
      const uint32_t ord = cur.ord;
      const int x = s.strip * kTilePx + row;
      const bool valid = x < p.W;
      const int y = PNP_Y(s.y_b + o);
      const uint32_t sc_last = cur.sc0 + (uint32_t)(min(o + 1, s.j_last) - s.j_first);
      const uint32_t slot = ord % kAccRing;
      const uint32_t taddr = lane_base + slot * tap_n;
      TileCur nxt = cur;
      tile_next(nxt);
      if (last_mode) {
        const float r0 = lq_a[0], r1 = lq_a[1], r2 = lq_a[2];
        {
          TileCur n2 = nxt;
          if (n2.valid) tile_next(n2);
          lq_a[0] = lq_b[0];
          lq_a[1] = lq_b[1];
          lq_a[2] = lq_b[2];
          lq_fetch(n2, lq_b);
        }
        ewait(smem_u32(&misc->step_done[sc_last & (kStepRing - 1)]), (sc_last >> kStepShift) & 1, 9);
        tc_fence_after();
        float v[16];
        if (half == 0) {
          tmem_ld16(taddr, v);
          tmem_ld_wait();
        }
        tc_fence_before();
        acc_release(slot);
        if (valid && half == 0) {
          const long long o_off = (long long)s.n * p.of_sn + (long long)y * p.of_sy + x;
          const float o0 = v[0] + misc->bias[0] + r0, o1 = v[1] + misc->bias[1] + r1, o2 = v[2] + misc->bias[2] + r2;
          if (!kPar && p.out_u8) {
            uint8_t* op = reinterpret_cast<uint8_t*>(outf_g) + o_off;
            op[0] = (uint8_t)quant_u8(o0);
            op[p.of_sc] = (uint8_t)quant_u8(o1);
            op[2 * p.of_sc] = (uint8_t)quant_u8(o2);
          } else {
            float* op = outf_g + o_off;
            op[0] = o0;
            op[p.of_sc] = o1;
            op[2 * p.of_sc] = o2;
          }
        }
        cur = nxt;
        continue;
      }
      const bool tr = PNP_TRACING && blockIdx.x == 0 && ord < 64 && threadIdx.x == 64 && !PNP_DBG(128);
      float pf0 = 0.f, pf1 = 0.f, pf2 = 0.f;
      if (kPar && nxt.valid) {
        TileCur n2 = nxt;
        tile_next(n2);
        if (n2.valid) par_load(n2, pf0, pf1, pf2);
      }
      const uint32_t s_io = ior.slot;
      if (store_warp) {
        if (elect_one()) {
          tma_store_wait_read<1>();
          if (p.has_id && ord >= 2 && idc.valid) {
            load_id(idc, idr.slot);
            idr.advance();
            tile_next(idc);
          }
        }
        __syncwarp();
      }
      if (p.has_id) {
        ewait(smem_u32(&misc->id_full[s_io]), ior.phase, 8);
      } else {
        named_bar_sync(1, 256);
      }
      if (kPar && nxt.valid) {
        ewait(smem_u32(&misc->par_done), (ord + 1) & 1, 11);
      } else {
        ewait(smem_u32(&misc->step_done[sc_last & (kStepRing - 1)]), (sc_last >> kStepShift) & 1, 9);
      }
      tc_fence_after();
      if (tr) p.trace[ord * 8 + 3] = clock64();
      uint8_t* rowp = sgen + L.io + s_io * kTileBytes + row * 128;
      float v[32];
      if (PNP_DBG(4)) {
#pragma unroll
        for (int j = 0; j < 32; ++j) v[j] = 0.f;
      } else {
        tmem_ld16(taddr + half * 32, v);
        tmem_ld16(taddr + half * 32 + 16, v + 16);
        if (kPar && nxt.valid) {
          const uint32_t s_nx = (s_io + 1 == (uint32_t)n_io) ? 0u : s_io + 1;
          blend_store(sgen + L.io + s_nx * kTileBytes + row * 128, pn0, pn1, pn2);
        } else {
          tmem_ld_wait();
        }
      }
      tc_fence_before();
      acc_release(slot);
      if (kPar && nxt.valid) par_release();
#pragma unroll
      for (int gg = 0; gg < 2; ++gg) {
        const int g = half * 2 + gg;
        float* vv = v + gg * 16;
        if (kPar) {
          const float4* sc4 = reinterpret_cast<const float4*>(&misc->scale[g * 16]);
          const float4* bi4 = reinterpret_cast<const float4*>(&misc->bias[g * 16]);
#pragma unroll
          for (int j4 = 0; j4 < 4; ++j4) {
            const float4 sc = kScale ? sc4[j4] : make_float4(1.f, 1.f, 1.f, 1.f);
            const float4 bi = bi4[j4];
            vv[4 * j4 + 0] = fmaf(vv[4 * j4 + 0], sc.x, bi.x);
            vv[4 * j4 + 1] = fmaf(vv[4 * j4 + 1], sc.y, bi.y);
            vv[4 * j4 + 2] = fmaf(vv[4 * j4 + 2], sc.z, bi.z);
            vv[4 * j4 + 3] = fmaf(vv[4 * j4 + 3], sc.w, bi.w);
          }
        } else {
#pragma unroll
          for (int j = 0; j < 16; ++j)
            vv[j] = kScale ? fmaf(vv[j], scale_r[gg * 16 + j], bias_r[gg * 16 + j]) : vv[j] + bias_r[gg * 16 + j];
        }
        uint4* c0 = reinterpret_cast<uint4*>(rowp + (((2 * g) ^ sw) << 4));
        uint4* c1 = reinterpret_cast<uint4*>(rowp + (((2 * g + 1) ^ sw) << 4));
        if (p.has_id || kPar) {
          const uint4 i0 = *c0, i1 = *c1;
          const uint32_t iw[8] = {i0.x, i0.y, i0.z, i0.w, i1.x, i1.y, i1.z, i1.w};
#pragma unroll
          for (int j = 0; j < 8; ++j) {
            vv[2 * j] += bf16_lo(iw[j]);
            vv[2 * j + 1] += bf16_hi(iw[j]);
          }
        }
#pragma unroll
        for (int j = 0; j < 16; ++j) vv[j] = act_fn(vv[j], p.act);
        uint4 o0, o1;
        o0.x = pack_bf16x2(vv[0], vv[1]);
        o0.y = pack_bf16x2(vv[2], vv[3]);
        o0.z = pack_bf16x2(vv[4], vv[5]);
        o0.w = pack_bf16x2(vv[6], vv[7]);
        o1.x = pack_bf16x2(vv[8], vv[9]);
        o1.y = pack_bf16x2(vv[10], vv[11]);
        o1.z = pack_bf16x2(vv[12], vv[13]);
        o1.w = pack_bf16x2(vv[14], vv[15]);
        if (!PNP_DBG(2)) {
          *c0 = o0;
          *c1 = o1;
        }
      }
      if (tr) p.trace[ord * 8 + 4] = clock64();
      fence_proxy_async_smem();
      named_bar_sync(2, 256);
      if (tr) p.trace[ord * 8 + 5] = clock64();
      if (store_warp) {
        if (elect_one()) {
          if (!PNP_DBG(2)) {
            if (!phantom(s)) {
              if (p.l2_out)
                tma_store_4d_hint(&p.tm_out, io_smem + s_io * kTileBytes, 0, s.strip * kTilePx, y, s.n + out_f,
                                  p.l2_out == 2 ? l2_policy_evict_last() : l2_policy_evict_first());
              else
                tma_store_4d(&p.tm_out, io_smem + s_io * kTileBytes, 0, s.strip * kTilePx, y, s.n + out_f);
            }
            tma_store_commit();
          }
        }
        __syncwarp();
      }
      ior.advance();
      if (kPar) {
        pn0 = pf0;
        pn1 = pf1;
        pn2 = pf2;
      }
      cur = nxt;
    }
    if (store_warp) {
      if (elect_one()) tma_store_wait_all<0>();
      __syncwarp();
    }
    }
  }

  tc_fence_before();
  if (kPair) cluster_sync_all(); else __syncthreads();
  if (PNP_TRACING && threadIdx.x == 0) {
    p.trace[2048 + blockIdx.x] += clock64();
    p.trace[2368 + blockIdx.x] = (long long)globaltimer_ns();
  }
  if (warp == 0) {
    tc_fence_after();
    if (kPair) tmem_dealloc2(tmem_base, kTmemCols);
    else tmem_dealloc(tmem_base, kTmemCols);
  }
}

#undef PNP_Y

size_t conv_rows_smem_bytes(const ConvParams& p) {
  const int full = 3 * 3 * p.tap_n * 128;
  const int w_bytes = p.pair ? full + (p.aux_k16 > 0 ? kWChunkBytes / 2 : 0) + (p.has_par ? 3 * 64 * 128 / 2 : 0)
                             : full + (p.aux_k16 > 0 ? kWChunkBytes : 0) + (p.has_par ? 3 * 64 * 128 : 0);
  return rows_layout(w_bytes, p.s_a, p.aux_k16 > 0, p.n_io).total + 1024;
}

namespace {
constexpr int kMaxSmem = 232448;

template <bool kPar, bool kScale, bool kPair>
cudaError_t launch_rows_variant(const ConvParams& p, int grid, size_t smem, cudaStream_t stream) {
  cudaLaunchConfig_t cfg = {};
  cfg.gridDim = dim3(grid);
  cfg.blockDim = dim3(kPar ? kRowsThreadsPar : kRowsThreads);
  cfg.dynamicSmemBytes = smem;
  cfg.stream = stream;
  cudaLaunchAttribute attr[2];
  attr[0].id = cudaLaunchAttributeProgrammaticStreamSerialization;
  attr[0].val.programmaticStreamSerializationAllowed = 1;
  cfg.attrs = attr;
  cfg.numAttrs = 1;
  if (kPair) {
    attr[1].id = cudaLaunchAttributeClusterDimension;
    attr[1].val.clusterDim.x = 2;
    attr[1].val.clusterDim.y = 1;
    attr[1].val.clusterDim.z = 1;
    cfg.numAttrs = 2;
  }
  return cudaLaunchKernelEx(&cfg, conv3x3_rows_kernel<kPar, kScale, kPair>, p);
}
template <bool kPar, bool kScale, bool kPair>
cudaError_t prepare_variant(int* max_pairs) {
  cudaError_t e = cudaFuncSetAttribute(conv3x3_rows_kernel<kPar, kScale, kPair>, cudaFuncAttributeMaxDynamicSharedMemorySize,
                                       kMaxSmem);
  if (e != cudaSuccess || !kPair) return e;
  cudaLaunchConfig_t cfg = {};
  cfg.gridDim = dim3(2 * 148);
  cfg.blockDim = dim3(kPar ? kRowsThreadsPar : kRowsThreads);
  cfg.dynamicSmemBytes = kMaxSmem;
  cudaLaunchAttribute attr[1];
  attr[0].id = cudaLaunchAttributeClusterDimension;
  attr[0].val.clusterDim.x = 2;
  attr[0].val.clusterDim.y = 1;
  attr[0].val.clusterDim.z = 1;
  cfg.attrs = attr;
  cfg.numAttrs = 1;
  int n = 0;
  e = cudaOccupancyMaxActiveClusters(&n, conv3x3_rows_kernel<kPar, kScale, kPair>, &cfg);
  if (e == cudaSuccess && n < *max_pairs) *max_pairs = n;
  return e;
}
}

cudaError_t conv_rows_prepare(int* max_pairs) {
  cudaError_t e;
  int pairs = 1 << 30;
  if ((e = prepare_variant<true, true, false>(&pairs)) != cudaSuccess) return e;
  if ((e = prepare_variant<true, false, false>(&pairs)) != cudaSuccess) return e;
  if ((e = prepare_variant<false, true, false>(&pairs)) != cudaSuccess) return e;
  if ((e = prepare_variant<false, false, false>(&pairs)) != cudaSuccess) return e;
  if ((e = prepare_variant<true, true, true>(&pairs)) != cudaSuccess) return e;
  if ((e = prepare_variant<true, false, true>(&pairs)) != cudaSuccess) return e;
  if ((e = prepare_variant<false, true, true>(&pairs)) != cudaSuccess) return e;
  if ((e = prepare_variant<false, false, true>(&pairs)) != cudaSuccess) return e;
  if (max_pairs) *max_pairs = pairs == (1 << 30) ? 0 : pairs;
  return cudaSuccess;
}

cudaError_t launch_conv_rows(const ConvParams& p, int grid, cudaStream_t stream) {
  const size_t smem = conv_rows_smem_bytes(p);
  const bool par = p.has_par != 0, scale = (p.scale != nullptr);
  if (p.pair) {
    if (par) return scale ? launch_rows_variant<true, true, true>(p, grid, smem, stream)
                          : launch_rows_variant<true, false, true>(p, grid, smem, stream);
    return scale ? launch_rows_variant<false, true, true>(p, grid, smem, stream)
                 : launch_rows_variant<false, false, true>(p, grid, smem, stream);
  }
  if (par) return scale ? launch_rows_variant<true, true, false>(p, grid, smem, stream)
                        : launch_rows_variant<true, false, false>(p, grid, smem, stream);
  return scale ? launch_rows_variant<false, true, false>(p, grid, smem, stream)
               : launch_rows_variant<false, false, false>(p, grid, smem, stream);
}

}
```

### pnpvcve_b200/engine.py

```python
import ctypes
import os

import numpy as np
import torch
import torch.nn.functional as F

from . import _lib, ops
from .ops import PNP_ACT_LRELU, PNP_ACT_NONE, PNP_ACT_RELU

SLICE_I, SLICE_P = 73, 80
ROW_BYTES = 9 * 64 * 128
WORK = ("kw", "pa", "pb", "xa", "xb", "t", "hr", "zero")


def key_schedule(key_row):
    t = len(key_row)
    bwd, fwd = [-1] * t, [-1] * t
    nxt = -1
    for i in range(t - 1, -1, -1):
        bwd[i] = nxt
        if key_row[i]:
            nxt = i
    prv = -1
    for i in range(t):
        fwd[i] = prv
        if key_row[i]:
            prv = i
    return bwd, fwd


def keyframe_rows(slices_host):
    key = (slices_host == SLICE_I) | (slices_host == SLICE_P)
    key[:, 0] = True
    key[:, -1] = True
    return key.tolist()


def group_clips(key_rows, max_batch, batch=True):
    groups = []
    for b, row in enumerate(key_rows):
        if batch and groups and row == key_rows[groups[-1][0]] and groups[-1][1] - groups[-1][0] < max_batch:
            groups[-1][1] = b + 1
        else:
            groups.append([b, b + 1])
    return [tuple(g) for g in groups]


def step_variants(bwd_key, fwd_key):
    t = len(bwd_key)
    names = []
    for s in range(t):
        i = t - 1 - s
        names.append("b_last" if i == t - 1 else ("b_merged" if bwd_key[i] == i + 1 else "b_sep"))
    for i in range(t):
        names.append("f_first" if i == 0 else ("f_merged" if fwd_key[i] == i - 1 else "f_sep"))
    return names


class _Program:

    def __init__(self, n, t, h, w, dev, maxn, nb, vsr, table_steps, lr_once=False):
        self.key = (n, t, h, w, dev, maxn, nb, vsr, lr_once)
        self.n, self.t, self.h, self.w, self.dev, self.maxn, self.nb, self.vsr = n, t, h, w, dev, maxn, nb, vsr
        self.img_bytes = h * w * 128
        self.lr_once = lr_once
        self.lr = torch.zeros((t * n if lr_once else maxn, h, w, 32), dtype=torch.bfloat16, device=dev)
        self.lr_img_bytes = h * w * 64
        first_work = t * n
        self.pool_images = first_work + len(WORK) * maxn
        self.pool = torch.empty((self.pool_images, h, w, 64), dtype=torch.bfloat16, device=dev)
        self.feats = self.pool[: t * n].view(t, n, h, w, 64)
        self.work = {}
        for k, name in enumerate(WORK):
            f0 = first_work + k * maxn
            self.work[name] = (f0, self.pool[f0:f0 + maxn])
        self.work["zero"][1].zero_()
        if vsr:
            self.u1 = ops.new_feature(maxn, 2 * h, 2 * w, dev)
            self.u2 = ops.new_feature(maxn, 4 * h, 4 * w, dev)
            self.hr4 = ops.new_feature(maxn, 4 * h, 4 * w, dev)
        self.stride = 8 + 2 * nb + (8 if vsr else 0)
        self.table_steps = 0
        self.table = self.img_off = self.host_table = self.host_off = None
        self.nodes = {}
        self.graphs = {}
        self.ensure_table(table_steps)
        self.step_word = torch.zeros(1, dtype=torch.int32, device=dev)
        self.cap_stream = torch.cuda.Stream(device=dev)
        self.uploaded = None

    def ensure_table(self, steps):
        if steps <= self.table_steps:
            return
        steps = max(steps, 2 * self.t)
        self.release_graphs()
        self.nodes = {}
        self.table_steps = steps
        self.table = torch.zeros((steps, self.stride, _lib.DYN_ENTRY_WORDS), dtype=torch.int64, device=self.dev)
        self.img_off = torch.zeros((steps, self.maxn, 2), dtype=torch.int64, device=self.dev)
        self.host_table = torch.zeros((steps, self.stride, _lib.DYN_ENTRY_WORDS), dtype=torch.int64).pin_memory()
        self.host_off = torch.zeros((steps, self.maxn, 2), dtype=torch.int64).pin_memory()

    def release_graphs(self):
        graphs, self.graphs = getattr(self, "graphs", {}), {}
        if graphs:
            lib = _lib.load()
            for g in graphs.values():
                lib.pnp_graph_destroy(g)

    def __del__(self):
        try:
            self.release_graphs()
        except Exception:
            pass


class BaeEngine:

    def __init__(self, module):
        self.m = module
        self.static_key = None
        self.static = None
        self.mix_slots = {}
        self.mix_pool = None
        self.prog = None
        self.launch_count = 0
        self.last_mode = "graph"
        self._done = None
        self.prof = None
        self.prof_every = 1
        self.use_graphs = os.environ.get("PNP_GRAPHS", "1") != "0"
        self.batch_clips = os.environ.get("PNP_BATCH_CLIPS", "1") != "0"
        self.lr_once = {"0": False, "1": True}.get(os.environ.get("PNP_LR_ONCE", ""), None)
        self.max_batch = 16

    def _param_key(self):
        return tuple((id(p), p._version, p.device, p.data_ptr()) for p in self.m.parameters())

    def invalidate(self):
        self.static = self.static_key = None
        self.mix_slots = {}

    def __getstate__(self):
        return {"m": self.m}

    def __setstate__(self, state):
        self.__init__(state["m"])

    def _pack_static(self, dev):
        key = self._param_key()
        if self.static is not None and self.static_key == key:
            return self.static
        m = self.m
        nb = m.num_blocks
        st = {}

        def f32(p):
            return p.detach().to(dev, torch.float32).contiguous()

        conv1_w = torch.zeros((2 * nb, ROW_BYTES), dtype=torch.uint8, device=dev)
        conv1_b, c2w, c2b, w1x1 = [], [], [], []
        for br, (name, branch) in enumerate((("bwd", m.backward_resblocks), ("fwd", m.forward_resblocks))):
            w_in = f32(branch.input_conv[0].weight)
            st[name + "_in_bias"] = f32(branch.input_conv[0].bias)
            def pack(in_begin, in_begin2=-1, with_aux=False, w_in=w_in):
                buf = ops.new_wpack_rowstack(dev, with_aux=with_aux)
                ops.pack_conv3x3_rowstack(w_in, buf, in_begin=in_begin, in_begin2=in_begin2, in_count=64)
                if with_aux:
                    ops.pack_aux(w_in, buf[ROW_BYTES:])
                return buf
            if name == "bwd":
                st["bwd_key_aux"] = pack(3, with_aux=True)
                st["bwd_merged_aux"] = pack(3, 67, with_aux=True)
                st["bwd_nb"] = pack(67)
            else:
                st["fwd_bf_aux"] = pack(131, with_aux=True)
                st["fwd_key"] = pack(3)
                st["fwd_merged"] = pack(3, 67)
                st["fwd_nb"] = pack(67)
            for k, blk in enumerate(branch.main):
                ops.pack_conv3x3_rowstack(f32(blk.conv1.weight), conv1_w[br * nb + k], flip_ky=True)
                conv1_b.append(f32(blk.conv1.bias))
                c2w.append(f32(blk.conv2.weight))
                c2b.append(f32(blk.conv2.bias))
                w1x1.append(torch.stack([f32(c.weight).view(64, 64) for c in
                                         (blk.conv16x16, blk.conv16x8, blk.conv8x8)], 0))
        st["conv1_w"] = conv1_w
        st["conv1_b"] = torch.stack(conv1_b, 0).contiguous()
        st["conv2_w_all"] = torch.stack(c2w, 0).contiguous()
        st["w1x1_all"] = torch.stack(w1x1, 0).contiguous()
        st["conv2_bias_all"] = torch.stack(c2b, 0).contiguous()
        hr = ops.new_wpack_rowstack(dev)
        ops.pack_conv3x3_rowstack(f32(m.conv_hr.weight), hr)
        st["hr_w"], st["hr_b"] = hr, f32(m.conv_hr.bias)
        last = ops.new_wpack_rowstack(dev, tap_n=16)
        ops.pack_conv3x3_rowstack(f32(m.conv_last.weight), last, tap_n=16)
        st["last_w"], st["last_b"] = last, f32(m.conv_last.bias)
        if m.vsr:
            for name, mod in (("up1", m.upsample1), ("up2", m.upsample2)):
                w_up, b_up = f32(mod.upsample_conv.weight), f32(mod.upsample_conv.bias)
                packs, biases = [], []
                for g in range(4):
                    buf = ops.new_wpack_rowstack(dev)
                    ops.pack_conv3x3_rowstack(w_up[g::4].contiguous(), buf)
                    packs.append(buf)
                    biases.append(b_up[g::4].contiguous())
                st[name + "_w"], st[name + "_b"] = packs, biases
        st["caa"] = dict(b0w=f32(m.BasePredictor.BaseNet[0].weight), b0b=f32(m.BasePredictor.BaseNet[0].bias),
                         b2w=f32(m.BasePredictor.BaseNet[2].weight), b2b=f32(m.BasePredictor.BaseNet[2].bias),
                         s0w=f32(m.BiasePredictor.fc[0].weight), s2w=f32(m.BiasePredictor.fc[2].weight))
        st["nb"] = nb
        self.static, self.static_key = st, key
        self.mix_slots = {}
        return st

    def _mix_slots_for(self, st, conds, experts, gamma, dev):
        nb2 = 2 * st["nb"]
        pool = self.mix_pool
        if pool is not None and (pool.device != dev or pool.shape[1] != nb2):
            pool = self.mix_pool = None
            self.mix_slots = {}
        need = [c for c in conds if c not in self.mix_slots]
        cap = 0 if pool is None else pool.shape[0]
        if len(self.mix_slots) + len(need) > cap:
            if len(conds) > cap:
                self.mix_pool = None
                self.mix_pool = torch.empty((max(48, 2 * len(conds)), nb2, ops.PACK_A_BYTES), dtype=torch.uint8, device=dev)
            self.mix_slots = {}
            need = list(conds)
        for c in need:
            slot = len(self.mix_slots)
            f = conds[c]
            ops.pack_mix_blocks(st["conv2_w_all"], st["w1x1_all"], experts[f], gamma[f], self.mix_pool[slot])
            self.mix_slots[c] = slot
        return self.mix_slots

    def _program(self, n, t, h, w, dev, maxn, steps):
        extra = t * n * h * w * 64
        lr_once = self.lr_once if self.lr_once is not None else \
            extra <= torch.cuda.get_device_properties(dev).total_memory // 8
        key = (n, t, h, w, dev, maxn, self.m.num_blocks, bool(self.m.vsr), lr_once)
        if self.prog is None or self.prog.key != key:
            self.prog = None
            self.prog = _Program(n, t, h, w, dev, maxn, self.m.num_blocks, bool(self.m.vsr), steps, lr_once)
        self.prog.ensure_table(steps)
        return self.prog

    def _build_nodes(self, pg, variant, nn, per_image, sparse, shapes, out_u8=False):
        lib = _lib.load()
        nodes = []
        h, w, nb = pg.h, pg.w, pg.nb
        pool_ptr = pg.pool.data_ptr()

        def dyn(node):
            r = _lib.DynRef()
            r.table, r.step, r.node, r.stride = pg.table.data_ptr(), pg.step_word.data_ptr(), node, pg.stride
            return r

        def conv(label, aux=False, idt=False, bias=False, par=False, act=PNP_ACT_NONE, flip=False, last=False,
                 image=False, src=None, out=None, hh=h, ww=w, lq_up4=False):
            d = ops.ConvDesc()
            d.src = src.data_ptr() if src is not None else pool_ptr
            d.src_images = 0 if src is not None else pg.pool_images
            d.aux, d.aux_images = (pg.lr.data_ptr(), pg.lr.shape[0]) if aux else (None, 0)
            d.aux_channels = 32 if aux else 0
            d.idt, d.idt_images = (pool_ptr, pg.pool_images) if idt else (None, 0)
            d.out_spx = d.out_sy = d.out_sn = 0
            if last:
                d.out, d.out_images = None, 0
            elif out is not None:
                d.out, d.out_images = out.data_ptr(), 0
                if not out.is_contiguous():
                    d.out_sn, d.out_sy, d.out_spx = out.stride(0), out.stride(1), out.stride(2)
            else:
                d.out, d.out_images = pool_ptr, pg.pool_images
            d.wpack, d.scale = None, None
            d.bias = 1 if bias else None
            if par:
                d.par = 1
                d.par_sn, d.par_sc, d.par_sy = shapes["par"]
            if last:
                d.lq, d.outf = 1, 1
                d.lq_sn, d.lq_sc, d.lq_sy = shapes["lq"]
                d.of_sn, d.of_sc, d.of_sy = shapes["outf"]
                d.out_u8 = 1 if out_u8 else 0
            d.N, d.H, d.W = nn, hh, ww
            d.tap_n = 16 if last else 64
            d.aux_k16 = 2 if aux else 0
            d.act, d.mode = act, (ops.PNP_CONV_LAST if last else ops.PNP_CONV_BF16)
            d.flip_y = 1 if flip else 0
            d.lq_up4 = 1 if lq_up4 else 0
            d.par_sparse = 1 if (par and sparse) else 0
            d.wpack_stable = 1
            d.per_image = 1 if image else 0
            d.img_off = None
            d.dyn = dyn(len(nodes))
            nodes.append(("conv", label, (lib.pnp_conv3x3, ctypes.byref(d), d)))

        def im2col():
            r = dyn(len(nodes))
            sn, sc, sy = shapes["lq"]
            nodes.append(("im2col", "im2col", (lib.pnp_lr_im2col_dyn, ctypes.byref(r), r, sn, sc, sy, nn, h, w, 32)))

        def warp():
            r = dyn(len(nodes))
            fsy, fsn = shapes["flow"]
            nodes.append(("warp", "warp", (lib.pnp_mv_warp_dyn, ctypes.byref(r), r, ctypes.c_void_p(pool_ptr), pg.pool_images,
                                           fsy, fsn, nn, h, w)))

        bwd = variant.startswith("b_")
        if bwd or not pg.lr_once:
            im2col()
        if variant not in ("b_last", "f_first"):
            warp()
        if variant in ("b_last", "b_merged", "f_first"):
            conv("input", aux=True, bias=True, act=PNP_ACT_LRELU)
        elif variant in ("b_sep", "f_merged"):
            conv("input", aux=True, bias=True)
            conv("input", idt=True, act=PNP_ACT_LRELU)
        else:
            conv("input", aux=True, bias=True)
            conv("input", idt=True)
            conv("input", idt=True, act=PNP_ACT_LRELU)
        for _ in range(nb):
            conv("block_a", bias=True, par=True, act=PNP_ACT_RELU, image=per_image)
            conv("block_b", idt=True, bias=True, flip=True)
        if not bwd:
            if pg.vsr:
                u1, u2, hr4 = pg.u1[:nn], pg.u2[:nn], pg.hr4[:nn]
                for g in range(4):
                    conv("up", bias=True, act=PNP_ACT_LRELU, out=u1[:, g >> 1::2, g & 1::2, :])
                for g in range(4):
                    conv("up", bias=True, act=PNP_ACT_LRELU, src=u1, out=u2[:, g >> 1::2, g & 1::2, :], hh=2 * h, ww=2 * w)
                conv("hr", bias=True, act=PNP_ACT_LRELU, src=u2, out=hr4, hh=4 * h, ww=4 * w)
                conv("last", bias=True, last=True, src=hr4, hh=4 * h, ww=4 * w, lq_up4=True)
            else:
                conv("hr", bias=True, act=PNP_ACT_LRELU)
                conv("last", bias=True, last=True)
        assert len(nodes) <= pg.stride
        return nodes

    def _fill_table(self, pg, st, g_idx, b0, nn, variants, bwd_key, fwd_key, slot_of, ptrs, per_image):
        t, n, nb, h, w = pg.t, pg.n, pg.nb, pg.h, pg.w
        tab = pg.host_table.numpy()[g_idx * 2 * t:(g_idx + 1) * 2 * t]
        off = pg.host_off.numpy()[g_idx * 2 * t:(g_idx + 1) * 2 * t]
        tab[:] = 0
        off[:] = 0
        steps = np.arange(2 * t)
        frame = np.where(steps < t, t - 1 - steps, steps - t)
        var = np.array(variants)
        img = pg.img_bytes
        pool_ptr = pg.pool.data_ptr()
        work = {k: v[0] for k, v in pg.work.items()}
        feats = lambda i: i * n + b0
        bk, fk = np.array(bwd_key), np.array(fwd_key)
        up = 4 if pg.vsr else 1
        plane = h * w * 4
        lr_ptr = ptrs["lrs"] + (b0 * t + frame) * 3 * plane
        par_ptr = ptrs["par"] + (b0 * t + frame) * 3 * plane
        outf_ptr = ptrs["out"] + (b0 * t + frame) * 3 * h * w * up * up * ptrs["out_elem"]
        mv_base = ptrs["mvs"] + (b0 * t + frame) * 4 * plane
        flow_x = np.where(steps < t, mv_base + 2 * plane, mv_base)
        bias_row = 2 * nb * 64
        slots = slot_of[b0:b0 + nn][:, frame]
        slot_stride = self.mix_pool.stride(0)
        if per_image:
            off[:, :nn, 0] = (slots * slot_stride).T
            off[:, :nn, 1] = (((b0 + np.arange(nn))[:, None] * t + frame[None, :]) * bias_row).T
            w_base = np.full(2 * t, self.mix_pool.data_ptr(), dtype=np.int64)
            b_base = np.full(2 * t, ptrs["bias_tab"], dtype=np.int64)
            off_ptr = pg.img_off.data_ptr() + (g_idx * 2 * t + steps) * pg.maxn * 16
        else:
            w_base = self.mix_pool.data_ptr() + slots[0] * slot_stride
            b_base = ptrs["bias_tab"] + (b0 * t + frame) * bias_row * 4
            off_ptr = np.zeros(2 * t, dtype=np.int64)

        def put(sel, node, p=(), i=(0, 0, 0, 0)):
            for k, v in enumerate(p):
                tab[sel, node, k] = v[sel] if isinstance(v, np.ndarray) else v
            iv = [np.asarray(x[sel] if isinstance(x, np.ndarray) else x, dtype=np.int64) & 0xFFFFFFFF for x in i]
            tab[sel, node, 6] = iv[0] | (iv[1] << 32)
            tab[sel, node, 7] = iv[2] | (iv[3] << 32)

        W = {k: v.data_ptr() for k, v in st.items() if isinstance(v, torch.Tensor)}
        lr64 = (frame * n + b0) if pg.lr_once else np.zeros(2 * t, dtype=np.int64)
        for v in set(variants):
            sel = var == v
            bwd = v.startswith("b_")
            br = 0 if bwd else 1
            node = 0
            if bwd or not pg.lr_once:
                put(sel, node, p=(lr_ptr, pg.lr.data_ptr() + lr64 * pg.lr_img_bytes))
                node += 1
            cur = feats(frame)
            if v not in ("b_last", "f_first"):
                kidx = np.where(steps < t, bk[frame], fk[frame])
                put(sel, node, p=(0, flow_x, flow_x + plane, 0), i=(feats(kidx), 0, 0, work["kw"]))
                node += 1
            in_bias = W["bwd_in_bias"] if bwd else W["fwd_in_bias"]
            if v == "b_last":
                put(sel, node, p=(W["bwd_merged_aux"], in_bias), i=(work["zero"], lr64, 0, work["xa"]))
                node += 1
            elif v == "b_merged":
                put(sel, node, p=(W["bwd_merged_aux"], in_bias), i=(work["kw"], lr64, 0, work["xa"]))
                node += 1
            elif v == "b_sep":
                put(sel, node, p=(W["bwd_key_aux"], in_bias), i=(work["kw"], lr64, 0, work["pa"]))
                put(sel, node + 1, p=(W["bwd_nb"],), i=(feats(frame + 1), 0, work["pa"], work["xa"]))
                node += 2
            elif v == "f_first":
                put(sel, node, p=(W["fwd_bf_aux"], in_bias), i=(cur, lr64, 0, work["xa"]))
                node += 1
            elif v == "f_merged":
                put(sel, node, p=(W["fwd_bf_aux"], in_bias), i=(cur, lr64, 0, work["pa"]))
                put(sel, node + 1, p=(W["fwd_merged"],), i=(work["kw"], 0, work["pa"], work["xa"]))
                node += 2
            else:
                put(sel, node, p=(W["fwd_bf_aux"], in_bias), i=(cur, lr64, 0, work["pa"]))
                put(sel, node + 1, p=(W["fwd_key"],), i=(work["kw"], 0, work["pa"], work["pb"]))
                put(sel, node + 2, p=(W["fwd_nb"],), i=(feats(frame - 1), 0, work["pb"], work["xa"]))
                node += 3
            x, other = work["xa"], work["xb"]
            for k in range(nb):
                blk = br * nb + k
                put(sel, node, p=(w_base + blk * ops.PACK_A_BYTES, b_base + blk * 256, par_ptr, 0, 0, off_ptr),
                    i=(x, 0, 0, work["t"]))
                o = cur if k == nb - 1 else other
                put(sel, node + 1, p=(W["conv1_w"] + blk * ROW_BYTES, W["conv1_b"] + blk * 256),
                    i=(work["t"], 0, x, o))
                node += 2
                x, other = o, x
            if not bwd:
                if pg.vsr:
                    for name, src_f in (("up1", cur), ("up2", 0)):
                        for g in range(4):
                            put(sel, node, p=(st[name + "_w"][g].data_ptr(), st[name + "_b"][g].data_ptr()),
                                i=(src_f, 0, 0, 0))
                            node += 1
                    put(sel, node, p=(W["hr_w"], W["hr_b"]), i=(0, 0, 0, 0))
                    put(sel, node + 1, p=(W["last_w"], W["last_b"], 0, lr_ptr, outf_ptr), i=(0, 0, 0, 0))
                else:
                    put(sel, node, p=(W["hr_w"], W["hr_b"]), i=(cur, 0, 0, work["hr"]))
                    put(sel, node + 1, p=(W["last_w"], W["last_b"], 0, lr_ptr, outf_ptr), i=(work["hr"], 0, 0, 0))

    @torch.no_grad()
    def forward(self, lrs, *args, **kwargs):
        dev = lrs.device
        if dev.type != "cuda":
            raise RuntimeError("pnpvcve_b200 runs on sm_100 CUDA devices only; there is no CPU fallback")
        with torch.cuda.device(dev):
            stream = torch.cuda.current_stream(dev)
            if self._done is not None and self._done[0] == dev:
                stream.wait_event(self._done[1])
            res = self._forward(lrs, *args, **kwargs)
            ev = self._done[1] if (self._done is not None and self._done[0] == dev) else torch.cuda.Event()
            ev.record(stream)
            self._done = (dev, ev)
        return res

    def _forward(self, lrs, QPs, slices, mvs, base_QPs, par_map, return_features=False, cond_host=None,
                 frame_ready=None, frame_done=None, out=None):
        m = self.m
        dev = lrs.device
        lib = _lib.load()
        _lib.require_device()
        n, t, c, h_in, w_in = lrs.shape
        assert h_in >= 64 and w_in >= 64, (
            f"The height and width of inputs should be at least 64, but got {h_in} and {w_in}.")
        pad_h, pad_w = (4 - h_in % 4) % 4, (4 - w_in % 4) % 4
        lq_u8 = lrs.dtype == torch.uint8
        if frame_ready is not None and (pad_h or pad_w or lq_u8 or not (lrs.is_contiguous() and mvs.is_contiguous()
                                                                       and par_map.is_contiguous())):
            for i in range(t):
                frame_ready(i)
            frame_ready = None
        if lq_u8:
            src = lrs if lrs.stride(-1) == 1 else lrs.contiguous()
            try:
                src.view(n * t, c, h_in, w_in)
            except RuntimeError:
                src = src.contiguous()
            lrs = ops.unit_from_u8(src, torch.empty(lrs.shape, dtype=torch.float32, device=dev))
        if pad_h or pad_w:
            lrs = F.pad(lrs.reshape(-1, c, h_in, w_in), [0, pad_w, 0, pad_h], mode="reflect")
            lrs = lrs.view(n, t, c, h_in + pad_h, w_in + pad_w)
        h, w = lrs.shape[3:]
        if tuple(mvs.shape) != (n, t, 4, h, w) or tuple(par_map.shape) != (n, t, 3, h, w):
            raise ValueError(f"The spatial sizes of input ({(h, w)}) and flow ({tuple(mvs.shape[3:])})"
                             f" / partition map ({tuple(par_map.shape[3:])}) are not the same.")
        lrs = lrs.contiguous().float()
        mvs = mvs.contiguous().float()
        par_map = par_map.contiguous().float()

        st = self._pack_static(dev)
        if cond_host is not None:
            cond = torch.stack([torch.as_tensor(c, dtype=torch.float32).reshape(n, t).cpu() for c in cond_host], 0)
        else:
            cond = torch.stack([slices.reshape(n, t).float(), base_QPs.reshape(n, t).float(),
                                QPs.reshape(n, t).float()], 0).cpu()
        key_rows = keyframe_rows(cond[0])
        crf_host, qp_host = cond[1].numpy(), cond[2].numpy()

        experts, gamma = ops.caa_heads(base_QPs.reshape(-1).float().contiguous(),
                                       QPs.reshape(-1).float().contiguous(), st["caa"], m.num_experts)
        bias_tab = ops.mix_bias(st["conv2_bias_all"], experts, gamma)
        conds, cond_keys = {}, []
        for b in range(n):
            row = [(float(crf_host[b, i]), float(qp_host[b, i])) for i in range(t)]
            cond_keys.append(row)
            for i, k in enumerate(row):
                conds.setdefault(k, b * t + i)
        slot_map = self._mix_slots_for(st, conds, experts, gamma, dev)
        slot_of = np.array([[slot_map[k] for k in row] for row in cond_keys], dtype=np.int64)

        groups = group_clips(key_rows, self.max_batch, self.batch_clips)
        maxn = max(b1 - b0 for b0, b1 in groups)
        pg = self._program(n, t, h, w, dev, maxn, 2 * t * len(groups))
        up = 4 if m.vsr else 1
        if out is None:
            out = torch.empty((n, t, 3, up * h, up * w), dtype=torch.float32, device=dev)
        elif tuple(out.shape) != (n, t, 3, up * h, up * w) or out.dtype not in (torch.float32, torch.uint8) or \
                out.device != dev or not out.is_contiguous():
            raise ValueError(f"out must be a contiguous fp32 or uint8 {(n, t, 3, up * h, up * w)} tensor on {dev}")
        out_u8 = out.dtype == torch.uint8
        feats = pg.feats
        bwd_feats = torch.empty_like(feats) if return_features else None
        sparse = bool(m.sparse_val) and not m.training

        if pg.uploaded is not None:
            pg.uploaded.synchronize()
        ptrs = dict(lrs=lrs.data_ptr(), par=par_map.data_ptr(), mvs=mvs.data_ptr(), out=out.data_ptr(),
                    out_elem=out.element_size(), bias_tab=bias_tab.data_ptr())
        plans = []
        for g_idx, (b0, b1) in enumerate(groups):
            bwd_key, fwd_key = key_schedule(key_rows[b0])
            variants = step_variants(bwd_key, fwd_key)
            per_image = bool((slot_of[b0:b1] != slot_of[b0:b0 + 1]).any())
            self._fill_table(pg, st, g_idx, b0, b1 - b0, variants, bwd_key, fwd_key, slot_of, ptrs, per_image)
            plans.append((b0, b1, variants, per_image))
        rows = 2 * t * len(groups)
        ops.fetch_pinned(pg.table[:rows], pg.host_table[:rows])
        ops.fetch_pinned(pg.img_off[:rows], pg.host_off[:rows])
        pg.uploaded = torch.cuda.Event()
        pg.uploaded.record()

        plane = h * w
        shapes = dict(lq=(t * 3 * plane, plane, w), par=(t * 3 * plane, plane, w), flow=(w, t * 4 * plane),
                      outf=(t * 3 * plane * up * up, plane * up * up, w * up))
        prof = self.prof
        graphs = self.use_graphs and prof is None
        self.last_mode = "graph" if graphs else "eager"
        seen = {}
        stream = ctypes.c_void_p(torch.cuda.current_stream().cuda_stream)
        step_ptr = ctypes.c_void_p(pg.step_word.data_ptr())
        launches = 0

        def phase(name):
            ev = torch.cuda.Event(enable_timing=True)
            ev.record()
            prof["phases"].append((name, ev))

        def run_nodes(nodes, stream):
            for kind, label, a in nodes:
                timed = prof is not None and label in prof
                if timed:
                    k = seen.get(label, 0)
                    seen[label] = k + 1
                    timed = (k % self.prof_every) == 0
                if timed:
                    e0 = torch.cuda.Event(enable_timing=True)
                    e1 = torch.cuda.Event(enable_timing=True)
                    e0.record()
                if kind == "conv":
                    rc = a[0](a[1], stream)
                elif kind == "warp":
                    rc = a[0](a[1], a[3], a[4], a[5], a[6], a[7], a[8], a[9], stream)
                else:
                    rc = a[0](a[1], a[3], a[4], a[5], a[6], a[7], a[8], a[9], stream)
                if timed:
                    e1.record()
                    prof[label].append((e0, e1))
                if rc != 0:
                    _lib.check(rc, "pnp_" + kind)

        def run_step(step, variant, nn, per_image):
            nonlocal launches
            key = (variant, nn, per_image, sparse, out_u8)
            nodes = pg.nodes.get(key)
            if nodes is None:
                nodes = pg.nodes[key] = self._build_nodes(pg, variant, nn, per_image, sparse, shapes, out_u8)
            launches += len(nodes)
            if not graphs:
                _lib.check(lib.pnp_set_step(step_ptr, step, stream), "pnp_set_step")
                if prof is not None and "phases" in prof:
                    n_in = sum(1 for k in nodes if k[1] in ("im2col", "warp", "input"))
                    n_blk = sum(1 for k in nodes if k[1] in ("block_a", "block_b"))
                    tag = "bwd" if variant.startswith("b_") else "fwd"
                    phase(tag + "_start")
                    run_nodes(nodes[:n_in], stream)
                    phase(tag + "_input_done")
                    run_nodes(nodes[n_in:n_in + n_blk], stream)
                    phase(tag + "_stack_done")
                    run_nodes(nodes[n_in + n_blk:], stream)
                    if tag == "fwd":
                        phase("fwd_head_done")
                else:
                    run_nodes(nodes, stream)
                return
            g = pg.graphs.get(key)
            if g is None:
                cap = ctypes.c_void_p(pg.cap_stream.cuda_stream)
                _lib.check(lib.pnp_graph_begin(cap), "pnp_graph_begin")
                handle = ctypes.c_void_p()
                try:
                    run_nodes(nodes, cap)
                finally:
                    rc = lib.pnp_graph_end(cap, ctypes.byref(handle))
                _lib.check(rc, "pnp_graph_end")
                g = pg.graphs[key] = handle
            rc = lib.pnp_graph_launch(g, step_ptr, step, stream)
            if rc != 0:
                _lib.check(rc, "pnp_graph_launch")

        for g_idx, (b0, b1, variants, per_image) in enumerate(plans):
            nn = b1 - b0
            base = g_idx * 2 * t
            for s in range(t):
                if frame_ready is not None:
                    frame_ready(t - 1 - s)
                run_step(base + s, variants[s], nn, per_image)
            if return_features:
                bwd_feats[:, b0:b1].copy_(feats[:, b0:b1])
            for i in range(t):
                run_step(base + t + i, variants[t + i], nn, per_image)
                if frame_done is not None and b1 == n:
                    frame_done(i, out)
        self.launch_count = launches
        if return_features:
            return out, bwd_feats.transpose(0, 1), feats.clone().transpose(0, 1)
        return out
```

### pnpvcve_b200/ops.py

```python
import ctypes

import torch

from . import _lib
from ._lib import (PNP_ACT_LRELU, PNP_ACT_NONE, PNP_ACT_RELU, PNP_CONV_BF16,
                   PNP_CONV_LAST, ConvDesc, DynRef)

CHUNK_BYTES = 8192


def _stream():
    return ctypes.c_void_p(torch.cuda.current_stream().cuda_stream)


def _on_device_of(fn):
    import functools

    @functools.wraps(fn)
    def wrapped(t, *args, **kwargs):
        if not t.is_cuda:
            raise ValueError(f"{fn.__name__}: CUDA tensors only (there is no CPU path)")
        if t.device.index == torch.cuda.current_device():
            return fn(t, *args, **kwargs)
        with torch.cuda.device(t.device):
            return fn(t, *args, **kwargs)
    return wrapped


def _ptr(t):
    return ctypes.c_void_p(t.data_ptr()) if t is not None else ctypes.c_void_p(0)


def _feat_check(t, name, strided=False):
    ok = t.dtype == torch.bfloat16 and t.dim() == 4 and t.shape[-1] == 64
    if ok and not t.is_contiguous():
        ok = strided and t.stride(3) == 1 and all(st % 8 == 0 and st > 0 for st in t.stride()[:3])
    if not ok:
        raise ValueError(f"{name} must be a contiguous bf16 (N,H,W,64) tensor, got "
                         f"{tuple(t.shape)} {t.dtype}")
    if not t.is_cuda:
        raise ValueError(f"{name} must live on a CUDA device")


def _plane_view_check(t, name):
    if t.dtype != torch.float32 or t.stride(-1) != 1 or not t.is_cuda:
        raise ValueError(f"{name} must be an fp32 CUDA view with unit innermost stride")


def _frames_view(t, name, dtype):
    if t.dtype != dtype or not t.is_cuda or t.dim() not in (4, 5) or t.shape[-3] != 3 or t.stride(-1) != 1:
        raise ValueError(f"{name} must be a {dtype} CUDA (F,3,H,W) or (n,T,3,H,W) view with unit innermost stride, got "
                         f"{tuple(t.shape)} {t.dtype}")
    if t.dim() == 5:
        try:
            t = t.view(-1, *t.shape[2:])
        except RuntimeError:
            raise ValueError(f"{name}: the (n,T) dimensions of a 5-D view must merge into one frame stride") from None
    return t


@_on_device_of
def unit_from_u8(src_u8, dst_f32):
    if src_u8.shape != dst_f32.shape:
        raise ValueError(f"unit_from_u8: shapes {tuple(src_u8.shape)} / {tuple(dst_f32.shape)} differ")
    s = _frames_view(src_u8, "src_u8", torch.uint8)
    d = _frames_view(dst_f32, "dst_f32", torch.float32)
    if s.numel() == 0:
        return dst_f32
    f, _, h, w = s.shape
    lib = _lib.load()
    _lib.check(lib.pnp_unit_from_u8(_ptr(s), s.stride(0), s.stride(1), s.stride(2), _ptr(d), d.stride(0), d.stride(1),
                                    d.stride(2), f, h, w, _stream()), "pnp_unit_from_u8")
    return dst_f32


def fetch_pinned(dst, src):
    nbytes = src.numel() * src.element_size()
    if not src.is_pinned() or not dst.is_cuda or not dst.is_contiguous() or not src.is_contiguous() or \
            dst.numel() * dst.element_size() != nbytes:
        raise ValueError("fetch_pinned: dst must be a contiguous CUDA tensor and src a pinned host tensor of the same size")
    with torch.cuda.device(dst.device):
        _lib.check(_lib.load().pnp_fetch_pinned(_ptr(dst), _ptr(src), nbytes, _stream()), "pnp_fetch_pinned")


def new_feature(n, h, w, device, zero=False):
    f = torch.zeros if zero else torch.empty
    return f((n, h, w, 64), dtype=torch.bfloat16, device=device)


@_on_device_of
def mv_warp(src, flow, dst, debug=False):
    _feat_check(src, "src")
    _feat_check(dst, "dst")
    _plane_view_check(flow, "flow")
    n, h, w, _ = src.shape
    if flow.dim() == 3:
        flow = flow.unsqueeze(0)
    if tuple(flow.shape) != (n, 2, h, w) or dst.shape != src.shape:
        raise ValueError(f"The spatial sizes of input ({(h, w)}) and flow ({tuple(flow.shape[-2:])}) "
                         "are not the same.")
    dx = dy = None
    if debug:
        if n != 1:
            raise ValueError("mv_warp: debug tap outputs need N == 1")
        dx = torch.empty((h, w), dtype=torch.int32, device=src.device)
        dy = torch.empty((h, w), dtype=torch.int32, device=src.device)
    lib = _lib.load()
    _lib.check(lib.pnp_mv_warp(_ptr(src), _ptr(flow[0, 0]), _ptr(flow[0, 1]), flow.stride(2), flow.stride(0),
                               _ptr(dst), n, h, w, _ptr(dx), _ptr(dy), _stream()), "pnp_mv_warp")
    return (dx, dy) if debug else None


def _aux_check(t, name):
    if not (t.dtype == torch.bfloat16 and t.dim() == 4 and t.shape[-1] in (32, 64) and t.is_contiguous() and t.is_cuda):
        raise ValueError(f"{name} must be a contiguous bf16 (N,H,W,64) or (N,H,W,32) CUDA tensor, got "
                         f"{tuple(t.shape)} {t.dtype}")


@_on_device_of
def lr_im2col(lr, dst):
    _plane_view_check(lr, "lr")
    _aux_check(dst, "dst")
    n, c, h, w = lr.shape
    if c != 3 or tuple(dst.shape[:3]) != (n, h, w):
        raise ValueError("lr_im2col: shape mismatch")
    lib = _lib.load()
    _lib.check(lib.pnp_lr_im2col(_ptr(lr), lr.stride(0), lr.stride(1), lr.stride(2), _ptr(dst), n, h, w,
                                 int(dst.shape[3]), _stream()), "pnp_lr_im2col")


def rowstack_bytes(tap_n=64, with_aux=False, with_par=False):
    return 9 * tap_n * 128 + (CHUNK_BYTES if with_aux else 0) + (3 * CHUNK_BYTES if with_par else 0)


def new_wpack_rowstack(device, tap_n=64, with_aux=False, with_par=False):
    n = (rowstack_bytes(tap_n, with_aux, with_par) + 1023) // 1024 * 1024
    return torch.zeros(n, dtype=torch.uint8, device=device)


@_on_device_of
def pack_conv3x3_rowstack(w, dst, coef=None, in_begin=0, in_begin2=-1, in_count=None, tap_n=64,
                          row_scale=None, flip_ky=False):
    if w.dtype != torch.float32 or not w.is_contiguous():
        raise ValueError("pack_conv3x3_rowstack: w must be contiguous fp32")
    if w.dim() == 4:
        e, (o, i) = 1, w.shape[:2]
    else:
        e, o, i = w.shape[:3]
    in_count = i - in_begin if in_count is None else in_count
    lib = _lib.load()
    _lib.check(lib.pnp_pack_conv3x3_rowstack(_ptr(w), e, _ptr(coef), _ptr(row_scale), o, i, in_begin, in_begin2,
                                             in_count,
                                             _ptr(dst), tap_n, int(flip_ky), _stream()), "pnp_pack_conv3x3_rowstack")


@_on_device_of
def pack_rows(w2d, dst, row_offset):
    if w2d.dtype != torch.float32 or w2d.dim() != 2:
        raise ValueError("pack_rows: need an fp32 matrix")
    lib = _lib.load()
    _lib.check(lib.pnp_pack_rows(_ptr(w2d), w2d.shape[0], w2d.shape[1], w2d.stride(0), w2d.stride(1),
                                 _ptr(dst), row_offset, _stream()), "pnp_pack_rows")


@_on_device_of
def pack_aux(w, dst):
    if w.dtype != torch.float32 or not w.is_contiguous() or w.dim() != 4:
        raise ValueError("pack_aux: w must be contiguous fp32 (O,I,3,3)")
    lib = _lib.load()
    _lib.check(lib.pnp_pack_aux(_ptr(w), w.shape[0], w.shape[1], _ptr(dst), _stream()), "pnp_pack_aux")


PACK_A_BYTES = 12 * CHUNK_BYTES


@_on_device_of
def pack_mix_blocks(w2, w1x1, coef, row_scale, dst):
    b, e = w2.shape[:2]
    if w2.dtype != torch.float32 or w1x1.dtype != torch.float32 or not w2.is_contiguous() or not w1x1.is_contiguous() \
            or tuple(w2.shape[2:]) != (64, 64, 3, 3) or tuple(w1x1.shape) != (b, 3, 64, 64):
        raise ValueError("pack_mix_blocks: need contiguous fp32 (B,E,64,64,3,3) and (B,3,64,64)")
    if dst.dtype != torch.uint8 or dst.dim() != 2 or dst.shape[0] != b or dst.shape[1] < PACK_A_BYTES or dst.stride(1) != 1:
        raise ValueError("pack_mix_blocks: dst must be uint8 (B, >= PACK_A_BYTES)")
    lib = _lib.load()
    _lib.check(lib.pnp_pack_mix_blocks(_ptr(w2), _ptr(w1x1), b, e, _ptr(coef), _ptr(row_scale), _ptr(dst),
                                       dst.stride(0), _stream()), "pnp_pack_mix_blocks")


@_on_device_of
def caa_heads(base_qp, qp, params, n_experts):
    f = base_qp.numel()
    dev = base_qp.device
    experts = torch.empty((f, n_experts), dtype=torch.float32, device=dev)
    gamma = torch.empty((f, 64), dtype=torch.float32, device=dev)
    lib = _lib.load()
    _lib.check(lib.pnp_caa_heads(_ptr(base_qp), _ptr(qp), f, _ptr(params["b0w"]), _ptr(params["b0b"]),
                                 _ptr(params["b2w"]), _ptr(params["b2b"]), _ptr(params["s0w"]),
                                 _ptr(params["s2w"]), n_experts, params["s0w"].numel(), _ptr(experts),
                                 _ptr(gamma), _stream()), "pnp_caa_heads")
    return experts, gamma


@_on_device_of
def mix_bias(conv2_bias, experts, gamma):
    b, e, _ = conv2_bias.shape
    f = experts.shape[0]
    out = torch.empty((f, b, 64), dtype=torch.float32, device=experts.device)
    lib = _lib.load()
    _lib.check(lib.pnp_mix_bias(_ptr(conv2_bias), b, e, _ptr(experts), _ptr(gamma), f, _ptr(out),
                                _stream()), "pnp_mix_bias")
    return out


def fill_conv_desc(d, src, wpack, out=None, aux=None, idt=None, scale=None, bias=None, par=None,
                   act=PNP_ACT_NONE, lq=None, outf=None, flip_y=False, wpack_stable=False,
                   lq_up4=False, par_sparse=False, img_off=None):
    n, h, w, _ = src.shape
    last = outf is not None
    d.src, d.aux, d.idt = src.data_ptr(), (aux.data_ptr() if aux is not None else None), \
        (idt.data_ptr() if idt is not None else None)
    d.out = out.data_ptr() if out is not None else None
    if out is not None and not out.is_contiguous():
        d.out_sn, d.out_sy, d.out_spx = out.stride(0), out.stride(1), out.stride(2)
    else:
        d.out_sn = d.out_sy = d.out_spx = 0
    d.lq_up4 = 1 if lq_up4 else 0
    d.par_sparse = 1 if (par_sparse and par is not None) else 0
    d.wpack = wpack.data_ptr()
    d.scale = scale.data_ptr() if scale is not None else None
    d.bias = bias.data_ptr() if bias is not None else None
    if par is not None:
        d.par, d.par_sn, d.par_sc, d.par_sy = par.data_ptr(), par.stride(0), par.stride(1), par.stride(2)
    else:
        d.par, d.par_sn, d.par_sc, d.par_sy = None, 0, 0, 0
    d.out_u8 = 0
    if last:
        d.lq, d.lq_sn, d.lq_sc, d.lq_sy = lq.data_ptr(), lq.stride(0), lq.stride(1), lq.stride(2)
        d.outf, d.of_sn, d.of_sc, d.of_sy = outf.data_ptr(), outf.stride(0), outf.stride(1), outf.stride(2)
        d.out_u8 = 1 if outf.dtype == torch.uint8 else 0
    else:
        d.lq, d.lq_sn, d.lq_sc, d.lq_sy = None, 0, 0, 0
        d.outf, d.of_sn, d.of_sc, d.of_sy = None, 0, 0, 0
    d.N, d.H, d.W = n, h, w
    d.tap_n = 16 if last else 64
    d.aux_k16 = 2 if aux is not None else 0
    d.aux_channels = int(aux.shape[3]) if aux is not None else 0
    d.act = act
    d.mode = PNP_CONV_LAST if last else PNP_CONV_BF16
    d.flip_y = 1 if flip_y else 0
    d.wpack_stable = 1 if wpack_stable else 0
    d.per_image = 1 if img_off is not None else 0
    d.img_off = img_off.data_ptr() if img_off is not None else None
    d.dyn.table, d.dyn.step, d.dyn.node, d.dyn.stride = None, None, 0, 0
    d.src_images = d.aux_images = d.idt_images = d.out_images = 0
    return d


@_on_device_of
def conv3x3(src, wpack, out=None, aux=None, idt=None, scale=None, bias=None, par=None,
            act=PNP_ACT_NONE, lq=None, outf=None, flip_y=False, wpack_stable=False, lq_up4=False,
            par_sparse=False, img_off=None):
    _feat_check(src, "src")
    for t, nm in ((out, "out"), (idt, "idt")):
        if t is not None:
            _feat_check(t, nm, strided=(nm == "out"))
            if t.shape != src.shape:
                raise ValueError(f"conv3x3: {nm} shape {tuple(t.shape)} != src {tuple(src.shape)}")
    if aux is not None:
        _aux_check(aux, "aux")
        if aux.shape[:3] != src.shape[:3]:
            raise ValueError(f"conv3x3: aux shape {tuple(aux.shape)} does not match src {tuple(src.shape)}")
    for t, nm in ((par, "par"), (lq, "lq"), (outf, "outf")):
        if t is not None:
            if nm == "outf" and t.dtype == torch.uint8:
                if t.stride(-1) != 1 or not t.is_cuda:
                    raise ValueError("outf must be a CUDA view with unit innermost stride")
            else:
                _plane_view_check(t, nm)
            hw = tuple(src.shape[1:3])
            if nm == "lq" and lq_up4:
                hw = (src.shape[1] // 4, src.shape[2] // 4)
            if t.dim() != 4 or t.shape[1] != 3 or t.shape[0] != src.shape[0] or tuple(t.shape[2:]) != hw:
                raise ValueError(f"conv3x3: {nm} must be (N,3,H,W) matching src" + (" / 4" if hw[0] != src.shape[1] else ""))
    if img_off is not None and (img_off.dtype != torch.int64 or tuple(img_off.shape) != (src.shape[0], 2) or
                                not img_off.is_contiguous() or not img_off.is_cuda):
        raise ValueError("conv3x3: img_off must be a contiguous int64 (N,2) CUDA tensor")
    d = fill_conv_desc(ConvDesc(), src, wpack, out, aux, idt, scale, bias, par, act, lq, outf, flip_y,
                       wpack_stable, lq_up4, par_sparse, img_off)
    need = rowstack_bytes(d.tap_n, aux is not None, par is not None)
    if img_off is None and wpack.numel() < need:
        raise ValueError("conv3x3: packed weight buffer too small for this configuration")
    lib = _lib.load()
    _lib.check(lib.pnp_conv3x3(ctypes.byref(d), _stream()), "pnp_conv3x3")
    return out if outf is None else outf
```

Baseline: 299.2.

## Build LR im2col aux tiles in-kernel from lq instead of a separate pass

```diff
diff --git a/pnpvcve_b200/csrc/pnp_api.cu b/pnpvcve_b200/csrc/pnp_api.cu
--- a/pnpvcve_b200/csrc/pnp_api.cu
+++ b/pnpvcve_b200/csrc/pnp_api.cu
@@ -489,13 +489,17 @@
     if (!c->out || c->tap_n != 64) return fail(PNP_ERR_ARG, "pnp_conv3x3: PNP_CONV_BF16 needs out and tap_n=64");
     if (c->out == c->src && !table) return fail(PNP_ERR_ARG, "pnp_conv3x3: out must not alias src (halo rows)");
   }
-  if ((c->aux != nullptr) != (c->aux_k16 > 0) || c->aux_k16 < 0 || c->aux_k16 > 4)
+  const bool lr_build = c->aux_channels == 3;
+  const bool has_aux = c->aux != nullptr || lr_build;
+  if (lr_build && (c->aux || last || !c->lq || c->aux_k16 != 2 || c->flip_y))
+    return fail(PNP_ERR_ARG, "pnp_conv3x3: aux_channels = 3 needs lq, aux = NULL, aux_k16 = 2, PNP_CONV_BF16, no flip_y");
+  if (has_aux != (c->aux_k16 > 0) || c->aux_k16 < 0 || c->aux_k16 > 4)
     return fail(PNP_ERR_ARG, "pnp_conv3x3: aux / aux_k16 mismatch");
   const bool aux32 = c->aux && c->aux_channels == 32;
   if (c->aux && c->aux_channels != 0 && c->aux_channels != 64 && !aux32)
-    return fail(PNP_ERR_ARG, "pnp_conv3x3: aux_channels is 64 (or 0) or 32");
+    return fail(PNP_ERR_ARG, "pnp_conv3x3: aux_channels is 64 (or 0), 32, or 3 without aux");
   if (aux32 && c->aux_k16 > 2) return fail(PNP_ERR_ARG, "pnp_conv3x3: a 32-channel aux source carries K <= 32");
-  if (par && (c->aux || c->idt)) return fail(PNP_ERR_ARG, "pnp_conv3x3: par takes no aux / idt");
+  if (par && (has_aux || c->idt)) return fail(PNP_ERR_ARG, "pnp_conv3x3: par takes no aux / idt");
   if (c->act < 0 || c->act > 2) return fail(PNP_ERR_ARG, "pnp_conv3x3: bad act");
   const bool strided_out = c->out_spx != 0 || c->out_sy != 0 || c->out_sn != 0;
   if (strided_out && (last || c->out_spx < 64 || c->out_sy < c->out_spx * c->W || (c->N > 1 && c->out_sn < c->out_sy * c->H) ||
@@ -549,7 +553,7 @@
   p.tiles_total = (int)tiles;
   const long long cols = (long long)c->N * p.strips;
   const int pair_mode = g_pair_override >= 0 ? g_pair_override : kn.pair;
-  const bool pair_ok = pair_mode != 0 && !last && !aux32 && c->tap_n == 64 && d->max_pairs >= 8 && (!par || kn.par_split) &&
+  const bool pair_ok = pair_mode != 0 && !last && !aux32 && !lr_build && c->tap_n == 64 && d->max_pairs >= 8 && (!par || kn.par_split) &&
                        (c->per_image ? (p.strips % 2 == 0 && c->N <= d->max_pairs)
                                      : (cols % 2 == 0 || cols >= 15 || pair_mode == 2));
   int grid;
@@ -588,7 +592,8 @@
   }
   p.tap_n = c->tap_n;
   p.aux_k16 = c->aux_k16;
-  p.aux_pitch64 = aux32 ? 1 : 0;
+  p.aux_pitch64 = (aux32 || lr_build) ? 1 : 0;
+  p.lr_build = lr_build ? 1 : 0;
   p.has_id = c->idt != nullptr;
   p.act = c->act;
   p.mode = last ? pnp::kModeLast : pnp::kModeBf16;
@@ -607,10 +612,10 @@
   p.debug_skip = kn.debug_skip;
   p.trace = kn.trace;
   const long long budget = 232448 - 2048;
-  const long long w_bytes = ((long long)9 * c->tap_n * 128 + (c->aux ? pnp::kWChunkBytes : 0) / (p.pair ? 2 : 1) +
+  const long long w_bytes = ((long long)9 * c->tap_n * 128 + (has_aux ? pnp::kWChunkBytes : 0) / (p.pair ? 2 : 1) +
                              (par ? 3 * 64 * 128 : 0) / (p.pair ? 2 : 1) + 1023) & ~1023LL;
   auto fixed_bytes = [&](int n_io) {
-    return w_bytes + (c->aux ? 2 * pnp::kTileBytes : 0) + (long long)n_io * pnp::kTileBytes;
+    return w_bytes + (has_aux ? 2 * pnp::kTileBytes : 0) + (long long)n_io * pnp::kTileBytes;
   };
   p.n_io = 2;
   if (par) p.n_io = 3;
diff --git a/pnpvcve_b200/csrc/pnp_conv.cuh b/pnpvcve_b200/csrc/pnp_conv.cuh
--- a/pnpvcve_b200/csrc/pnp_conv.cuh
+++ b/pnpvcve_b200/csrc/pnp_conv.cuh
@@ -12,6 +12,7 @@
 constexpr int kWChunkBytes = 8192;
 constexpr int kRowsThreads = 352;
 constexpr int kRowsThreadsPar = 480;
+constexpr int kRowsThreadsLr = 384;
 constexpr int kEpilogueWarps = 8;
 constexpr int kMaxASlots = 8;
 constexpr int kMaxIoSlots = 6;
@@ -74,6 +75,7 @@
   long long* trace;
   int debug_skip;
   int out_u8;
+  int lr_build;
 };
 
 __device__ __forceinline__ void par_sparse_select(float& p0, float& p1, float& p2) {
diff --git a/pnpvcve_b200/csrc/pnp_conv_rows.cu b/pnpvcve_b200/csrc/pnp_conv_rows.cu
--- a/pnpvcve_b200/csrc/pnp_conv_rows.cu
+++ b/pnpvcve_b200/csrc/pnp_conv_rows.cu
@@ -23,6 +23,7 @@
 constexpr int kStepShift = PNP_STEP_RING_LOG2;
 constexpr int kStepRing = 1 << kStepShift;
 constexpr int kParCol = 320;
+constexpr int kAuxSlotsMax = 4;
 
 struct RowsLayout {
   uint32_t w, a, aux, io, misc, total;
@@ -47,7 +48,7 @@
   uint64_t step_done[kStepRing];
   uint64_t acc_free[kAccRingMax];
   uint64_t par_done;
-  uint64_t aux_full[2];
+  uint64_t aux_full[kAuxSlotsMax];
   uint64_t id_full[kMaxIoSlots];
   uint64_t io_empty[kMaxIoSlots];
   uint32_t tmem_base;
@@ -114,8 +115,8 @@
 
 }
 
-template <bool kPar, bool kScale, bool kPair>
-__global__ void __launch_bounds__(kPar ? kRowsThreadsPar : kRowsThreads, 1)
+template <bool kPar, bool kScale, bool kPair, bool kLr = false>
+__global__ void __launch_bounds__(kPar ? kRowsThreadsPar : (kLr ? kRowsThreadsLr : kRowsThreads), 1)
 conv3x3_rows_kernel(const __grid_constant__ ConvParams p) {
   constexpr int kAccRing = kPar ? 5 : 8;
   const int rank = kPair ? (int)cluster_ctarank() : 0;
@@ -176,7 +177,7 @@
       for (int i = 0; i < kMaxIoSlots; ++i) mbar_init(smem_u32(&misc->dy_full[i]), 4);
       misc->slot_free = 0;
       mbar_init(smem_u32(&misc->par_done), 1);
-      for (int i = 0; i < 2; ++i) mbar_init(smem_u32(&misc->aux_full[i]), 1);
+      for (int i = 0; i < kAuxSlotsMax; ++i) mbar_init(smem_u32(&misc->aux_full[i]), 1);
       for (int i = 0; i < kMaxIoSlots; ++i) {
         mbar_init(smem_u32(&misc->id_full[i]), 1);
         mbar_init(smem_u32(&misc->io_empty[i]), 1);
@@ -241,6 +242,9 @@
   const uint32_t a_smem = sbase + L.a;
   const uint32_t aux_smem = sbase + L.aux;
   const uint32_t io_smem = sbase + L.io;
+  const uint32_t aux_shift = (!kPair && p.aux_pitch64) ? 2u : 1u;
+  const uint32_t aux_mask = (1u << aux_shift) - 1u;
+  const uint32_t aux_slot_bytes = (!kPair && p.aux_pitch64) ? kTileBytes / 2 : kTileBytes;
 
   if (warp == 0) {
     if (elect_one()) {
@@ -248,7 +252,7 @@
       const uint64_t pol_src = p.l2_src == 2 ? l2_policy_evict_last() : l2_policy_evict_first();
       Ring ar(s_a);
       uint32_t sc = 0, ord = 0;
-      uint32_t aux_step[2] = {0, 0};
+      uint32_t aux_step[kAuxSlotsMax] = {0, 0, 0, 0};
       for (SegIter it(p, t_begin, t_end, rank); it.valid();) {
         const Segment s = it.get();
         const int x0 = s.strip * kTilePx;
@@ -271,13 +275,13 @@
             else
               tma_load_4d(a_smem + ar.slot * kASlotBytes, &p.tm_src, fb, 0, x0 - 1, PNP_Y(s.y_b + j), s.n + src_f);
           }
+          if (PNP_TRACING && blockIdx.x == 0 && sc < 64) p.trace[3328 + sc] = clock64();
           if (j >= 0 && j < s.len) {
-            if (p.aux_k16 > 0) {
-              const uint32_t as = ord & 1;
-              if (ord >= 2) {
-                const uint32_t ps = aux_step[as];
+            if (!kLr && p.aux_k16 > 0) {
+              const uint32_t as = ord & aux_mask;
+              const uint32_t ps = aux_step[as];
+              if ((ord >> aux_shift) > 0 && ps + (uint32_t)s_a > sc)
                 pwait(smem_u32(&misc->step_done[ps & (kStepRing - 1)]), (ps >> kStepShift) & 1, 2);
-              }
               aux_step[as] = sc;
               const uint32_t ab = smem_u32(&misc->aux_full[as]);
               if (kPair) {
@@ -285,8 +289,8 @@
                 tma_load_4d_pair(aux_smem + as * kTileBytes, &p.tm_aux, mapa_shared(ab, 0), 0, x0, PNP_Y(s.y_b + j),
                                  s.n + aux_f);
               } else {
-                mbar_arrive_expect_tx(ab, p.aux_pitch64 ? kTileBytes / 2 : kTileBytes);
-                tma_load_4d(aux_smem + as * kTileBytes, &p.tm_aux, ab, 0, x0, PNP_Y(s.y_b + j), s.n + aux_f);
+                mbar_arrive_expect_tx(ab, aux_slot_bytes);
+                tma_load_4d(aux_smem + as * aux_slot_bytes, &p.tm_aux, ab, 0, x0, PNP_Y(s.y_b + j), s.n + aux_f);
               }
             }
             ++ord;
@@ -506,7 +510,7 @@
             step_body([&](int dx, int k) { emit1(std::false_type{}, dx, k); });
         }
         if (p.aux_k16 > 0 && centre) {
-          const uint32_t a_lo = umma_desc_lo(aux_smem + (cur_od & 1) * kTileBytes);
+          const uint32_t a_lo = umma_desc_lo(aux_smem + (cur_od & aux_mask) * aux_slot_bytes);
           for (int k = 0; k < p.aux_k16; ++k) {
             if (kPair)
               umma2_bf16_lo<0>(tmem_base + (cur_od % kAccRing) * tap_n, a_lo + 2 * k, aux_w_lo + 2 * k,
@@ -554,7 +558,7 @@
           const bool centre = (j >= 0 && j < s.len);
           if (p.aux_k16 > 0 && centre) {
             const uint32_t od = ord0 + j;
-            mbar_wait(smem_u32(&misc->aux_full[od & 1]), (od >> 1) & 1, 7);
+            mbar_wait(smem_u32(&misc->aux_full[od & aux_mask]), (od >> aux_shift) & 1, 7);
           }
           st_release_shared(go_step, sc + 1);
           if (trs) p.trace[2560 + sc * 4 + 2] = clock64();
@@ -562,6 +566,85 @@
         ord0 += s.len;
         it.next(s);
       }
+    }
+  } else if (kLr && warp == 11) {
+    float win[3][3][5];
+    auto fetch = [&](float (&r)[3][5], const Segment& sg, int y) {
+      const int xb = sg.strip * kTilePx + lane;
+      const int xh = lane == 0 ? xb - 1 : xb + 3 * 32 + 1;
+      const bool row_ok = y >= 0 && y < p.H;
+      const float* src = lq_g + (long long)sg.n * p.lq_sn + (long long)y * p.lq_sy;
+#pragma unroll
+      for (int c = 0; c < 3; ++c) {
+#pragma unroll
+        for (int i = 0; i < 4; ++i) {
+          const int x = xb + 32 * i;
+          r[c][i] = (row_ok && x < p.W) ? __ldg(src + c * p.lq_sc + x) : 0.f;
+        }
+        r[c][4] = (row_ok && (lane == 0 || lane == 31) && xh >= 0 && xh < p.W) ? __ldg(src + c * p.lq_sc + xh) : 0.f;
+      }
+    };
+    uint32_t sc0 = 0, ord = 0;
+    uint32_t h0 = 0, h1 = 0, h2 = 0, h3 = 0;
+    for (SegIter it(p, t_begin, t_end, rank); it.valid();) {
+      const Segment s = it.get();
+      const int x0 = s.strip * kTilePx;
+      fetch(win[0], s, s.y_b - 1);
+      fetch(win[1], s, s.y_b);
+      fetch(win[2], s, s.y_b + 1);
+      for (int o = 0; o < s.len; ++o, ++ord) {
+        const uint32_t as = ord & aux_mask;
+        if (ord > aux_mask) ewait(smem_u32(&misc->step_done[h0 & (kStepRing - 1)]), (h0 >> kStepShift) & 1, 15);
+        float nx[3][5];
+        fetch(nx, s, o + 1 < s.len ? s.y_b + o + 2 : -1);
+        uint8_t* slot = sgen + L.aux + as * aux_slot_bytes;
+#pragma unroll
+        for (int i = 0; i < 4; ++i) {
+          const int px = lane + 32 * i;
+          float v[32];
+#pragma unroll
+          for (int ky = 0; ky < 3; ++ky) {
+#pragma unroll
+            for (int c = 0; c < 3; ++c) {
+              const float m = win[ky][c][i];
+              const float lsrc = i > 0 ? __shfl_sync(0xffffffffu, win[ky][c][i > 0 ? i - 1 : 0], 31) : win[ky][c][4];
+              const float rsrc = i < 3 ? __shfl_sync(0xffffffffu, win[ky][c][i < 3 ? i + 1 : 3], 0) : win[ky][c][4];
+              const float up = __shfl_up_sync(0xffffffffu, m, 1), dn = __shfl_down_sync(0xffffffffu, m, 1);
+              v[(3 * ky + 0) * 3 + c] = lane == 0 ? lsrc : up;
+              v[(3 * ky + 1) * 3 + c] = m;
+              v[(3 * ky + 2) * 3 + c] = lane == 31 ? rsrc : dn;
+            }
+          }
+#pragma unroll
+          for (int k = 27; k < 32; ++k) v[k] = 0.f;
+          if (x0 + px >= p.W) {
+#pragma unroll
+            for (int k = 0; k < 32; ++k) v[k] = 0.f;
+          }
+#pragma unroll
+          for (int q = 0; q < 4; ++q)
+            *reinterpret_cast<uint4*>(slot + px * 64 + ((q ^ ((px >> 1) & 3)) << 4)) =
+                make_uint4(pack_bf16x2(v[8 * q], v[8 * q + 1]), pack_bf16x2(v[8 * q + 2], v[8 * q + 3]),
+                           pack_bf16x2(v[8 * q + 4], v[8 * q + 5]), pack_bf16x2(v[8 * q + 6], v[8 * q + 7]));
+        }
+        fence_proxy_async_smem();
+        __syncwarp();
+        if (lane == 0) mbar_arrive(smem_u32(&misc->aux_full[as]));
+#pragma unroll
+        for (int c = 0; c < 3; ++c)
+#pragma unroll
+          for (int i = 0; i < 5; ++i) {
+            win[0][c][i] = win[1][c][i];
+            win[1][c][i] = win[2][c][i];
+            win[2][c][i] = nx[c][i];
+          }
+        h0 = h1;
+        h1 = h2;
+        h2 = h3;
+        h3 = sc0 + (uint32_t)(o - s.j_first);
+      }
+      sc0 += (uint32_t)(s.j_last - s.j_first + 1);
+      it.next(s);
     }
   } else if (warp >= 11 && !(kPar && p.par_split)) {
   } else {
@@ -1065,11 +1148,11 @@
 namespace {
 constexpr int kMaxSmem = 232448;
 
-template <bool kPar, bool kScale, bool kPair>
+template <bool kPar, bool kScale, bool kPair, bool kLr = false>
 cudaError_t launch_rows_variant(const ConvParams& p, int grid, size_t smem, cudaStream_t stream) {
   cudaLaunchConfig_t cfg = {};
   cfg.gridDim = dim3(grid);
-  cfg.blockDim = dim3(kPar ? kRowsThreadsPar : kRowsThreads);
+  cfg.blockDim = dim3(kPar ? kRowsThreadsPar : (kLr ? kRowsThreadsLr : kRowsThreads));
   cfg.dynamicSmemBytes = smem;
   cfg.stream = stream;
   cudaLaunchAttribute attr[2];
@@ -1084,12 +1167,12 @@
     attr[1].val.clusterDim.z = 1;
     cfg.numAttrs = 2;
   }
-  return cudaLaunchKernelEx(&cfg, conv3x3_rows_kernel<kPar, kScale, kPair>, p);
+  return cudaLaunchKernelEx(&cfg, conv3x3_rows_kernel<kPar, kScale, kPair, kLr>, p);
 }
-template <bool kPar, bool kScale, bool kPair>
+template <bool kPar, bool kScale, bool kPair, bool kLr = false>
 cudaError_t prepare_variant(int* max_pairs) {
-  cudaError_t e = cudaFuncSetAttribute(conv3x3_rows_kernel<kPar, kScale, kPair>, cudaFuncAttributeMaxDynamicSharedMemorySize,
-                                       kMaxSmem);
+  cudaError_t e = cudaFuncSetAttribute(conv3x3_rows_kernel<kPar, kScale, kPair, kLr>,
+                                       cudaFuncAttributeMaxDynamicSharedMemorySize, kMaxSmem);
   if (e != cudaSuccess || !kPair) return e;
   cudaLaunchConfig_t cfg = {};
   cfg.gridDim = dim3(2 * 148);
@@ -1120,6 +1203,8 @@
   if ((e = prepare_variant<true, false, true>(&pairs)) != cudaSuccess) return e;
   if ((e = prepare_variant<false, true, true>(&pairs)) != cudaSuccess) return e;
   if ((e = prepare_variant<false, false, true>(&pairs)) != cudaSuccess) return e;
+  if ((e = prepare_variant<false, true, false, true>(&pairs)) != cudaSuccess) return e;
+  if ((e = prepare_variant<false, false, false, true>(&pairs)) != cudaSuccess) return e;
   if (max_pairs) *max_pairs = pairs == (1 << 30) ? 0 : pairs;
   return cudaSuccess;
 }
@@ -1127,6 +1212,9 @@
 cudaError_t launch_conv_rows(const ConvParams& p, int grid, cudaStream_t stream) {
   const size_t smem = conv_rows_smem_bytes(p);
   const bool par = p.has_par != 0, scale = (p.scale != nullptr);
+  if (p.lr_build)
+    return scale ? launch_rows_variant<false, true, false, true>(p, grid, smem, stream)
+                 : launch_rows_variant<false, false, false, true>(p, grid, smem, stream);
   if (p.pair) {
     if (par) return scale ? launch_rows_variant<true, true, true>(p, grid, smem, stream)
                           : launch_rows_variant<true, false, true>(p, grid, smem, stream);
diff --git a/pnpvcve_b200/engine.py b/pnpvcve_b200/engine.py
--- a/pnpvcve_b200/engine.py
+++ b/pnpvcve_b200/engine.py
@@ -59,12 +59,13 @@
 
 class _Program:
 
-    def __init__(self, n, t, h, w, dev, maxn, nb, vsr, table_steps, lr_once=False):
+    def __init__(self, n, t, h, w, dev, maxn, nb, vsr, table_steps, lr_once=None):
         self.key = (n, t, h, w, dev, maxn, nb, vsr, lr_once)
         self.n, self.t, self.h, self.w, self.dev, self.maxn, self.nb, self.vsr = n, t, h, w, dev, maxn, nb, vsr
         self.img_bytes = h * w * 128
         self.lr_once = lr_once
-        self.lr = torch.zeros((t * n if lr_once else maxn, h, w, 32), dtype=torch.bfloat16, device=dev)
+        self.lr = None if lr_once is None else \
+            torch.zeros((t * n if lr_once else maxn, h, w, 32), dtype=torch.bfloat16, device=dev)
         self.lr_img_bytes = h * w * 64
         first_work = t * n
         self.pool_images = first_work + len(WORK) * maxn
@@ -236,9 +237,7 @@
         return self.mix_slots
 
     def _program(self, n, t, h, w, dev, maxn, steps):
-        extra = t * n * h * w * 64
-        lr_once = self.lr_once if self.lr_once is not None else \
-            extra <= torch.cuda.get_device_properties(dev).total_memory // 8
+        lr_once = self.lr_once
         key = (n, t, h, w, dev, maxn, self.m.num_blocks, bool(self.m.vsr), lr_once)
         if self.prog is None or self.prog.key != key:
             self.prog = None
@@ -257,13 +256,15 @@
             r.table, r.step, r.node, r.stride = pg.table.data_ptr(), pg.step_word.data_ptr(), node, pg.stride
             return r
 
+        lr_build = pg.lr_once is None
+
         def conv(label, aux=False, idt=False, bias=False, par=False, act=PNP_ACT_NONE, flip=False, last=False,
                  image=False, src=None, out=None, hh=h, ww=w, lq_up4=False):
             d = ops.ConvDesc()
             d.src = src.data_ptr() if src is not None else pool_ptr
             d.src_images = 0 if src is not None else pg.pool_images
-            d.aux, d.aux_images = (pg.lr.data_ptr(), pg.lr.shape[0]) if aux else (None, 0)
-            d.aux_channels = 32 if aux else 0
+            d.aux, d.aux_images = (pg.lr.data_ptr(), pg.lr.shape[0]) if (aux and not lr_build) else (None, 0)
+            d.aux_channels = (3 if lr_build else 32) if aux else 0
             d.idt, d.idt_images = (pool_ptr, pg.pool_images) if idt else (None, 0)
             d.out_spx = d.out_sy = d.out_sn = 0
             if last:
@@ -284,6 +285,9 @@
                 d.lq_sn, d.lq_sc, d.lq_sy = shapes["lq"]
                 d.of_sn, d.of_sc, d.of_sy = shapes["outf"]
                 d.out_u8 = 1 if out_u8 else 0
+            elif aux and lr_build:
+                d.lq = 1
+                d.lq_sn, d.lq_sc, d.lq_sy = shapes["lq"]
             d.N, d.H, d.W = nn, hh, ww
             d.tap_n = 16 if last else 64
             d.aux_k16 = 2 if aux else 0
@@ -309,7 +313,7 @@
                                            fsy, fsn, nn, h, w)))
 
         bwd = variant.startswith("b_")
-        if bwd or not pg.lr_once:
+        if not lr_build and (bwd or not pg.lr_once):
             im2col()
         if variant not in ("b_last", "f_first"):
             warp()
@@ -383,13 +387,14 @@
             tab[sel, node, 7] = iv[2] | (iv[3] << 32)
 
         W = {k: v.data_ptr() for k, v in st.items() if isinstance(v, torch.Tensor)}
+        lr_build = pg.lr_once is None
         lr64 = (frame * n + b0) if pg.lr_once else np.zeros(2 * t, dtype=np.int64)
         for v in set(variants):
             sel = var == v
             bwd = v.startswith("b_")
             br = 0 if bwd else 1
             node = 0
-            if bwd or not pg.lr_once:
+            if not lr_build and (bwd or not pg.lr_once):
                 put(sel, node, p=(lr_ptr, pg.lr.data_ptr() + lr64 * pg.lr_img_bytes))
                 node += 1
             cur = feats(frame)
@@ -399,24 +404,24 @@
                 node += 1
             in_bias = W["bwd_in_bias"] if bwd else W["fwd_in_bias"]
             if v == "b_last":
-                put(sel, node, p=(W["bwd_merged_aux"], in_bias), i=(work["zero"], lr64, 0, work["xa"]))
+                put(sel, node, p=(W["bwd_merged_aux"], in_bias, 0, lr_ptr), i=(work["zero"], lr64, 0, work["xa"]))
                 node += 1
             elif v == "b_merged":
-                put(sel, node, p=(W["bwd_merged_aux"], in_bias), i=(work["kw"], lr64, 0, work["xa"]))
+                put(sel, node, p=(W["bwd_merged_aux"], in_bias, 0, lr_ptr), i=(work["kw"], lr64, 0, work["xa"]))
                 node += 1
             elif v == "b_sep":
-                put(sel, node, p=(W["bwd_key_aux"], in_bias), i=(work["kw"], lr64, 0, work["pa"]))
+                put(sel, node, p=(W["bwd_key_aux"], in_bias, 0, lr_ptr), i=(work["kw"], lr64, 0, work["pa"]))
                 put(sel, node + 1, p=(W["bwd_nb"],), i=(feats(frame + 1), 0, work["pa"], work["xa"]))
                 node += 2
             elif v == "f_first":
-                put(sel, node, p=(W["fwd_bf_aux"], in_bias), i=(cur, lr64, 0, work["xa"]))
+                put(sel, node, p=(W["fwd_bf_aux"], in_bias, 0, lr_ptr), i=(cur, lr64, 0, work["xa"]))
                 node += 1
             elif v == "f_merged":
-                put(sel, node, p=(W["fwd_bf_aux"], in_bias), i=(cur, lr64, 0, work["pa"]))
+                put(sel, node, p=(W["fwd_bf_aux"], in_bias, 0, lr_ptr), i=(cur, lr64, 0, work["pa"]))
                 put(sel, node + 1, p=(W["fwd_merged"],), i=(work["kw"], 0, work["pa"], work["xa"]))
                 node += 2
             else:
-                put(sel, node, p=(W["fwd_bf_aux"], in_bias), i=(cur, lr64, 0, work["pa"]))
+                put(sel, node, p=(W["fwd_bf_aux"], in_bias, 0, lr_ptr), i=(cur, lr64, 0, work["pa"]))
                 put(sel, node + 1, p=(W["fwd_key"],), i=(work["kw"], 0, work["pa"], work["pb"]))
                 put(sel, node + 2, p=(W["fwd_nb"],), i=(feats(frame - 1), 0, work["pb"], work["xa"]))
                 node += 3
diff --git a/pnpvcve_b200/ops.py b/pnpvcve_b200/ops.py
--- a/pnpvcve_b200/ops.py
+++ b/pnpvcve_b200/ops.py
@@ -214,7 +214,7 @@
 
 def fill_conv_desc(d, src, wpack, out=None, aux=None, idt=None, scale=None, bias=None, par=None,
                    act=PNP_ACT_NONE, lq=None, outf=None, flip_y=False, wpack_stable=False,
-                   lq_up4=False, par_sparse=False, img_off=None):
+                   lq_up4=False, par_sparse=False, img_off=None, aux_lr=None):
     n, h, w, _ = src.shape
     last = outf is not None
     d.src, d.aux, d.idt = src.data_ptr(), (aux.data_ptr() if aux is not None else None), \
@@ -240,11 +240,13 @@
         d.out_u8 = 1 if outf.dtype == torch.uint8 else 0
     else:
         d.lq, d.lq_sn, d.lq_sc, d.lq_sy = None, 0, 0, 0
+        if aux_lr is not None:
+            d.lq, d.lq_sn, d.lq_sc, d.lq_sy = aux_lr.data_ptr(), aux_lr.stride(0), aux_lr.stride(1), aux_lr.stride(2)
         d.outf, d.of_sn, d.of_sc, d.of_sy = None, 0, 0, 0
     d.N, d.H, d.W = n, h, w
     d.tap_n = 16 if last else 64
-    d.aux_k16 = 2 if aux is not None else 0
-    d.aux_channels = int(aux.shape[3]) if aux is not None else 0
+    d.aux_k16 = 2 if (aux is not None or aux_lr is not None) else 0
+    d.aux_channels = int(aux.shape[3]) if aux is not None else (3 if aux_lr is not None else 0)
     d.act = act
     d.mode = PNP_CONV_LAST if last else PNP_CONV_BF16
     d.flip_y = 1 if flip_y else 0
@@ -259,7 +261,7 @@
 @_on_device_of
 def conv3x3(src, wpack, out=None, aux=None, idt=None, scale=None, bias=None, par=None,
             act=PNP_ACT_NONE, lq=None, outf=None, flip_y=False, wpack_stable=False, lq_up4=False,
-            par_sparse=False, img_off=None):
+            par_sparse=False, img_off=None, aux_lr=None):
     _feat_check(src, "src")
     for t, nm in ((out, "out"), (idt, "idt")):
         if t is not None:
@@ -270,7 +272,9 @@
         _aux_check(aux, "aux")
         if aux.shape[:3] != src.shape[:3]:
             raise ValueError(f"conv3x3: aux shape {tuple(aux.shape)} does not match src {tuple(src.shape)}")
-    for t, nm in ((par, "par"), (lq, "lq"), (outf, "outf")):
+    if aux_lr is not None and aux is not None:
+        raise ValueError("conv3x3: aux and aux_lr exclude each other")
+    for t, nm in ((par, "par"), (lq, "lq"), (outf, "outf"), (aux_lr, "aux_lr")):
         if t is not None:
             if nm == "outf" and t.dtype == torch.uint8:
                 if t.stride(-1) != 1 or not t.is_cuda:
@@ -286,8 +290,8 @@
                                 not img_off.is_contiguous() or not img_off.is_cuda):
         raise ValueError("conv3x3: img_off must be a contiguous int64 (N,2) CUDA tensor")
     d = fill_conv_desc(ConvDesc(), src, wpack, out, aux, idt, scale, bias, par, act, lq, outf, flip_y,
-                       wpack_stable, lq_up4, par_sparse, img_off)
-    need = rowstack_bytes(d.tap_n, aux is not None, par is not None)
+                       wpack_stable, lq_up4, par_sparse, img_off, aux_lr)
+    need = rowstack_bytes(d.tap_n, d.aux_k16 > 0, par is not None)
     if img_off is None and wpack.numel() < need:
         raise ValueError("conv3x3: packed weight buffer too small for this configuration")
     lib = _lib.load()
```

New measurement: 301.8 (median of 6 runs). No clear change (+0.9%).
